# luotuoqingshan/SDPLRPlus.jl

Hardware: AMD Instinct MI355X
Metric: augmented-Lagrangian iters/sec + HBM GB/s, MaxCut n=1e5 r=32 (higher is better)
Workload: dtype f64

## Files before the change

sdplrplus.jl_amd/cabi.py:

```python
from __future__ import annotations

import ctypes as C
import os
from typing import Optional, Tuple

import numpy as np

OK = 0
ERR_INVALID_ARG = -1
ERR_HIP = -2
ERR_NOT_DESCENT = -3
ERR_STATE = -4
ERR_NO_DEVICE = -5
ERR_ALLOC = -6
ERR_UNSERVED = -7
MAJOR_RESUME = 2

F_RT, F_GT, F_DIRT, F_LBFGS_S, F_LBFGS_Y, F_SCRATCH = 0, 1, 2, 100, 200, 300
(V_LAMBDA, V_LAMBDA_UB, V_B, V_Y, V_PV_RAW, V_PV_LB, V_PV, V_A_RD, V_A_DD, V_LBFGS_RHO, V_LBFGS_A,
 V_UVT, V_TRIU_S_NZVAL, V_S_NZVAL, V_SCRATCH) = range(15)
STAT_NAMES = ("graph_captures", "graph_capture_failures", "graph_capture_skipped", "graph_batches",
              "eager_batches", "lanczos_graph_replays", "lanczos_eager_rounds", "inner_iterations",
              "resident_loops", "resident_lanczos", "resident_fg", "resident_shared_launches", "p_less_loops",
              "group_launch_loops", "ring_history_loops", "ring_materializations")
S_SIGMA, S_OBJ, S_LBFGS_LATEST = 0, 1, 2

_i32, _i64, _f64, _vp = C.c_int32, C.c_int64, C.c_double, C.c_void_p
_pi32, _pi64, _pf64 = C.POINTER(C.c_int32), C.POINTER(C.c_int64), C.POINTER(C.c_double)



class FgItem(C.Structure):
    _fields_ = [("s", _vp), ("normC", _f64), ("normb", _f64), ("gtol_relative", _i32), ("ptol_relative", _i32),
                ("lagrangian", _f64), ("grad_norm", _f64), ("primal_vio_norm", _f64), ("obj", _f64), ("status", _i32)]


class MajorItem(C.Structure):
    _fields_ = [("s", _vp), ("normC", _f64), ("normb", _f64), ("gtol_relative", _i32), ("ptol_relative", _i32),
                ("use_armijo", _i32), ("update_lambda", _i32), ("sigma", _f64), ("cur_gtol", _f64), ("fprec_eps", _f64),
                ("max_local_iters", _i64), ("time_budget_s", _f64), ("lagrangian", _f64), ("grad_norm", _f64),
                ("primal_vio_norm", _f64), ("last_alpha", _f64), ("obj", _f64), ("iters_done", _i64),
                ("exit_reason", _i32), ("status", _i32)]


class DualItem(C.Structure):
    _fields_ = [("s", _vp), ("trace_bound", _f64), ("iter", _i64), ("v0", _pf64), ("y_out", _pf64),
                ("dual_value", _f64), ("mineig", _f64), ("status", _i32)]


SIGNATURES = {
    "device_count": [_pi32],
    "set_device": [_i32],
    "last_error": [_vp],
    "version": [],
    "device_synchronize": [],
    "warmup": [_i32],
    "trim_pools": [],
    "create": [_i64, _i64, _i64, _i64, C.POINTER(_vp)],
    "set_sparse": [_vp, _i64, _i64, _pi64, _pi64, _pf64, _pf64, _pi64, _i64, _pi64, _pi64, _i64,
                   _pi64, _pi64, _pi64],
    "set_sparse_coo": [_vp, _i64, _i64, _pi64, _pi64, _pi64, _pf64, _pi64],
    "get_layout": [_vp, _i32, _pi64, _pf64, _i64, _pi64],
    "add_symlowrank": [_vp, _i64, _i64, _i64, _pf64, _pf64],
    "finalize": [_vp],
    "destroy": [_vp],
    "reset_rank": [_vp, _i64],
    "set_factor": [_vp, _i32, _pf64],
    "get_factor": [_vp, _i32, _pf64],
    "set_vec": [_vp, _i32, _pf64, _i64],
    "get_vec": [_vp, _i32, _pf64, _i64],
    "set_scalar": [_vp, _i32, _f64],
    "get_scalar": [_vp, _i32, _pf64],
    "get_dims": [_vp, _pi64, _pi64, _pi64, _pi64, _pi64, _pi64, _pi64],
    "A": [_vp, _i32, _i32, _i32],
    "At_preprocess": [_vp],
    "At_left": [_vp, _i32, _i32],
    "At_right": [_vp, _pf64, _pf64, _i64],
    "At_right_device": [_vp, _vp, _vp, _i64],
    "get_stats": [_vp, _pi64, _i32, _pi32],
    "S_eigval": [_vp, _i64, _i32, _i64, _f64, _i64, _pf64, _pf64, _pi64, _pi64],
    "factor_dot": [_vp, _i32, _i32, _pf64],
    "f": [_vp, _pf64],
    "g": [_vp],
    "fg": [_vp, _f64, _f64, _i32, _i32, _pf64, _pf64, _pf64],
    "lbfgs_clear": [_vp],
    "lbfgs_dir": [_vp, _i32, _pf64],
    "descent_fallback": [_vp],
    "lbfgs_update": [_vp, _f64],
    "linesearch": [_vp, _f64, _pf64, _pf64],
    "linesearch_armijo": [_vp, _f64, _pf64, _pf64],
    "axpy_R": [_vp, _f64],
    "norms": [_vp, _f64, _f64, _i32, _i32, _pf64, _pf64],
    "update_lambda": [_vp],
    "inner_loop": [_vp, _f64, _f64, _i32, _i32, _i32, _f64, _f64, _i64, _f64, _pf64, _pf64, _pf64,
                   _pf64, _pi64, _pi32],
    "major_iteration": [_vp, _f64, _f64, _i32, _i32, _i32, _i32, _f64, _f64, _f64, _i64, _f64, _pf64, _pf64, _pf64,
                        _pf64, _pi64, _pi32],
    "batch_fg": [_i32, C.POINTER(FgItem)],
    "batch_major_iteration": [_i32, C.POINTER(MajorItem)],
    "batch_dual_obj": [_i32, C.POINTER(DualItem)],
    "lanczos": [_vp, _i64, _pf64, _pf64, _pf64, _pi64],
    "tridiag_mineig": [_pf64, _pf64, _i64, _pf64],
    "approx_mineigval_lanczos": [_vp, _i64, _pf64, _pf64],
    "dual_obj": [_vp, _f64, _i64, _pf64, _pf64, _pf64],
    "profile_enable": [_vp, _i32],
    "profile_filter": [_vp, C.c_char_p],
    "profile_count": [_vp, _pi32],
# ... 420 lines not shown
```

sdplrplus.jl_amd/csrc/k_dense.h:

```cpp
#pragma once
#include "common.h"

struct FactorArena {
  double* base;
  long long stride;
  int h;
};
#define AS_R 0
#define AS_G 1
#define AS_D 2
#define AS_S0 3

#ifdef SDPLR_NO_NT
__device__ __forceinline__ double2 ldnt2(const double* p, long long i) { return reinterpret_cast<const double2*>(p)[i]; }
__device__ __forceinline__ void stnt2(double* p, long long i, double2 v) { reinterpret_cast<double2*>(p)[i] = v; }
#else
typedef double sdplr_d2 __attribute__((ext_vector_type(2)));
__device__ __forceinline__ double2 ldnt2(const double* p, long long i) {
  const sdplr_d2 t = __builtin_nontemporal_load(reinterpret_cast<const sdplr_d2*>(p) + i);
  double2 o;
  o.x = t.x;
  o.y = t.y;
  return o;
}
// ... 181 lines not shown
      return;
    }
    c.iters = iters + 1;
    c.lastval = Lcur;
  }
  int ord[H];
  {
    int j = latest - 1;
#pragma unroll
    for (int i = 0; i < H; i++) {
      ord[i] = j;
      j = (j <= 0) ? H - 1 : j - 1;
    }
  }
  double Sg_s[H], Yg_s[H];
#pragma unroll
  for (int l = 0; l < H; l++) {
    Sg_s[l] = c.Sg[l];
    Yg_s[l] = c.Yg[l];
  }
  double al_s[H], ga_s[H];
#pragma unroll
  for (int l = 0; l < H; l++) {
    al_s[l] = c.c_alpha[l];
    ga_s[l] = c.c_gamma[l];
  }
  if (do_coeff) {
    double SYp[H][H], YYp[H][H], Sgp[H], Ygp[H], rhop[H];
#pragma unroll
    for (int a = 0; a < H; a++) {
      Sgp[a] = c.Sg[ord[a]];
      Ygp[a] = c.Yg[ord[a]];
      rhop[a] = c.rho[ord[a]];
#pragma unroll
      for (int b = 0; b < H; b++) {
        SYp[a][b] = c.SY[ord[a] * SDPLR_HMAX + ord[b]];
        YYp[a][b] = c.YY[ord[a] * SDPLR_HMAX + ord[b]];
      }
    }
    double al[H], ga[H];
#pragma unroll
    for (int i = 0; i < H; i++) {
      double sq = Sgp[i];
#pragma unroll
      for (int k = 0; k < i; k++) sq -= al[k] * SYp[i][k];
      al[i] = rhop[i] * sq;
    }
#pragma unroll
    for (int i = H - 1; i >= 0; i--) {
      double yr = Ygp[i];
#pragma unroll
      for (int k = 0; k < H; k++) yr -= al[k] * YYp[i][k];
#pragma unroll
      for (int k = H - 1; k > i; k--) yr += ga[k] * SYp[k][i];
      const double beta = rhop[i] * yr;
      ga[i] = al[i] - beta;
    }
#pragma unroll
    for (int i = 0; i < H; i++) {
      c.a[ord[i]] = al[i];
      c.c_alpha[ord[i]] = al[i];
      c.c_gamma[ord[i]] = ga[i];
#pragma unroll
      for (int l = 0; l < H; l++)
        if (ord[i] == l) {
          al_s[l] = al[i];
          ga_s[l] = ga[i];
        }
    }
  }
  if (desc_mode) {
    const double g = grel ? gnorm * normC : gnorm;
    double d = norms ? nrm0 : g * g;
#pragma unroll
    for (int l = 0; l < H; l++) d -= al_s[l] * Yg_s[l];
#pragma unroll
    for (int l = 0; l < H; l++) d += ga_s[l] * Sg_s[l];
    if (desc_mode == 1) d = -d;
    c.descent = d;
    c.fallback = (isnan(d) || d >= 0.0) ? 1 : 0;
  }
}

__device__ __forceinline__ void lbfgs_boundary_body(DevCtrl* __restrict__ c, int h, int jfixed, int fin_mode, int do_loop, int do_coeff, int nb_partials, const double* __restrict__ partials, int desc_mode, double* __restrict__ pv_raw, int m) {
  __shared__ SeamLds gd;
  const int tid = threadIdx.x, wave = tid >> 6, lane = tid & 63;
#ifdef SDPLR_STAMPS
  const unsigned long long st0 = __builtin_amdgcn_s_memtime();
#endif
  const int gp = c->gram_pending, np = c->norms_pending;
  const int op = c->obj_pending;
  static_assert(sizeof(DevCtrl) / 8 <= 1024, "one word of the control block per thread");
  const unsigned long long cw = reinterpret_cast<const unsigned long long*>(c)[min(tid, (int)(sizeof(DevCtrl) / 8) - 1)];
  if (wave >= 14) {
    const int nbp = (wave == 14) ? c->nb_gnorm : c->nb_pvnorm;
    const double* p = slot_partials(partials, wave == 14 ? SLOT_GNORM2 : SLOT_PVNORM2);
    const double2* p2 = reinterpret_cast<const double2*>(p);
    double2 v[8];
#pragma unroll
    for (int u = 0; u < 8; u++) v[u] = p2[lane + 64 * u];
    double t = 0.0;
#pragma unroll
    for (int u = 0; u < 8; u++) {
      const int i = 2 * (lane + 64 * u);
      t += (i < nbp) ? v[u].x : 0.0;
      t += (i + 1 < nbp) ? v[u].y : 0.0;
    }
    for (int i = lane + 1024; i < nbp; i += 64) t += p[i];
    t = wave_sum(t);
    if (lane == 0) gd.nrm[wave - 14] = t;
  } else if (fin_mode != 0) {
    const int np2 = (nb_partials + 1) >> 1;
    for (int s0 = wave; s0 < 5 * h; s0 += 28) {
      const int s1 = s0 + 14;
      const bool two = s1 < 5 * h;
      const double2* pa = reinterpret_cast<const double2*>(slot_partials(partials, SLOT_GRAM + (s0 / h) * SDPLR_HMAX + s0 % h));
      const double2* pb = two ? reinterpret_cast<const double2*>(slot_partials(partials, SLOT_GRAM + (s1 / h) * SDPLR_HMAX + s1 % h)) : pa;
      double ta = 0.0, tb = 0.0;
#pragma unroll 4
      for (int i = lane; i < np2; i += 64) {
        const double2 a = pa[i], b = pb[i];
        const bool hi = 2 * i + 1 < nb_partials;
        ta += a.x;
        ta += hi ? a.y : 0.0;
        tb += b.x;
        tb += hi ? b.y : 0.0;
      }
      ta = wave_sum(ta);
      tb = wave_sum(tb);
      if (lane == 0) {
        gd.red[(s0 / h) * SDPLR_HMAX + s0 % h] = ta;
        if (two) gd.red[(s1 / h) * SDPLR_HMAX + s1 % h] = tb;
      }
    }
  }
  if (tid < (int)(sizeof(DevCtrl) / 8)) reinterpret_cast<unsigned long long*>(&gd.c)[tid] = cw;
  const bool fin = (fin_mode == 2) || (fin_mode == 1 && gp);
  const bool norms = np != 0;
  if (!fin && !do_coeff && !do_loop && !norms && !op) return;
  __syncthreads();
  if (tid == 0 && op) {
    gd.c.obj = gd.c.obj_next;
    gd.c.obj_pending = 0;
    if (pv_raw != nullptr) pv_raw[m] = gd.c.obj_next;
  }
  if (tid == 0 && fin_mode == 1 && gd.c.ring_on) {
    if (gp) {
      gd.c.ring_alpha[gd.c.latest % h] = gd.c.alpha;
      gd.c.ring_k = (gd.c.ring_k + 1) % (h + 1);
      gd.c.ring_n = min(gd.c.ring_n + 1, h);
    } else if (gd.c.reldelta_exit) {
      gd.c.ring_unc = 1;
    }
  }
#ifdef SDPLR_STAMPS
  const unsigned long long st1 = __builtin_amdgcn_s_memtime();
#endif
  if (tid == 0) {
    switch (h) {
      case 1: seam_serial_small<1>(gd, jfixed, fin_mode, do_loop, do_coeff, fin, norms, desc_mode); break;
      case 2: seam_serial_small<2>(gd, jfixed, fin_mode, do_loop, do_coeff, fin, norms, desc_mode); break;
      case 3: seam_serial_small<3>(gd, jfixed, fin_mode, do_loop, do_coeff, fin, norms, desc_mode); break;
      case 4: seam_serial_small<4>(gd, jfixed, fin_mode, do_loop, do_coeff, fin, norms, desc_mode); break;
      default: seam_serial(gd, h, jfixed, fin_mode, do_loop, do_coeff, fin, norms, desc_mode);
    }
  }
  __syncthreads();
#ifdef SDPLR_STAMPS
  const unsigned long long st2 = __builtin_amdgcn_s_memtime();
#endif
  {
    const unsigned long long* src = reinterpret_cast<const unsigned long long*>(&gd.c);
    unsigned long long* dst = reinterpret_cast<unsigned long long*>(c);
    for (int t = tid; t < (int)(sizeof(DevCtrl) / 8); t += 1024) dst[t] = src[t];
  }
#ifdef SDPLR_STAMPS
  asm volatile("s_waitcnt vmcnt(0)" ::: "memory");
  const unsigned long long st3 = __builtin_amdgcn_s_memtime();
  if (tid == 0 && do_loop && (gd.c.iters % 64) == 33) {
    printf("[seam] loads+sums %llu  serial %llu  store %llu (s_memtime ticks)\n", st1 - st0, st2 - st1, st3 - st2);
  }
#endif
}
__global__ void __launch_bounds__(1024)
k_lbfgs_boundary(DevCtrl* __restrict__ c, int h, int jfixed, int fin_mode, int do_loop, int do_coeff,
                 int nb_partials, const double* __restrict__ partials, int desc_mode, double* __restrict__ pv_raw = nullptr,
                 int m = 0) {
  lbfgs_boundary_body(c, h, jfixed, fin_mode, do_loop, do_coeff, nb_partials, partials, desc_mode, pv_raw, m);
}

template <int HM, bool NTH>
__device__ __forceinline__ void lbfgs_dir_body(const DevCtrl* __restrict__ c, FactorArena A, long long N, int h, int negate, int check_done, double* __restrict__ partials, int inline_fallback) {
  __shared__ double sh[8];
  const int dn = check_done ? c->done : 0;
  double* G = aslot(A, AS_G);
  double* dir = aslot(A, AS_D);
  const int latest = c->latest;
  const int fb = inline_fallback ? c->fallback : 0;
  int order[HM];
  double ca[HM], cg[HM];
  {
    int j = latest - 1;
#pragma unroll
    for (int i = 0; i < HM; i++) {
      order[i] = j;
      if (i < h) {
        ca[i] = c->c_alpha[j];
        cg[i] = c->c_gamma[j];
      } else {
        ca[i] = 0.0;
        cg[i] = 0.0;
      }
      j = (j <= 0) ? h - 1 : j - 1;
    }
  }
  double* ynext = (h > 0 && inline_fallback != 2) ? aslot(A, as_y0(A) + (latest % h)) : nullptr;
  const double sgn = negate ? -1.0 : 1.0;
  if (dn) return;
  double desc = 0.0;
  const long long N2 = N >> 1;
  const long long stride = (long long)gridDim.x * SDPLR_NT;
  const double* yp[HM];
  const double* sp_[HM];
#pragma unroll
  for (int k = 0; k < HM; k++) {
    const int slot = (k < h) ? order[k] : 0;
    yp[k] = (h > 0) ? aslot(A, as_y0(A) + slot) : G;
    sp_[k] = (h > 0) ? aslot(A, AS_S0 + slot) : G;
  }
  for (long long i = (long long)blockIdx.x * SDPLR_NT + threadIdx.x; i < N2; i += stride) {
    const double2 g = ldnt2(G, i);
    double2 yv[HM], sv[HM];
#pragma unroll
    for (int k = 0; k < HM; k++) {
      if constexpr (NTH) {
        yv[k] = ldnt2(yp[k], i);
        sv[k] = ldnt2(sp_[k], i);
      } else {
        yv[k] = reinterpret_cast<const double2*>(yp[k])[i];
        sv[k] = reinterpret_cast<const double2*>(sp_[k])[i];
      }
    }
    double2 r = g;
#pragma unroll
    for (int k = 0; k < HM; k++) {
      r.x -= ca[k] * yv[k].x;
      r.y -= ca[k] * yv[k].y;
    }
#pragma unroll
    for (int k = HM - 1; k >= 0; k--) {
      r.x += cg[k] * sv[k].x;
      r.y += cg[k] * sv[k].y;
    }
    double2 d;
    d.x = sgn * r.x;
    d.y = sgn * r.y;
    if (fb) {
      d.x = -g.x;
      d.y = -g.y;
      reinterpret_cast<double2*>(G)[i] = d;
    }
    reinterpret_cast<double2*>(dir)[i] = d;
    if (ynext) {
      double2 ng;
      ng.x = -g.x;
      ng.y = -g.y;
      stnt2(ynext, i, ng);
    }
    desc += d.x * g.x + d.y * g.y;
  }
  if ((N & 1) && blockIdx.x == 0 && threadIdx.x == 0) {
// ... 434 lines not shown
```

sdplrplus.jl_amd/csrc/k_group.h:

```cpp
#pragma once
#include "k_dense.h"
#include "k_scalar.h"
#include "k_sparse.h"

struct GrpSeamArgs {
  DevCtrl* c;
  int h, jfixed, fin_mode, do_loop, do_coeff, nb_partials;
  const double* partials;
  int desc_mode, m;
  double* pv_raw;
};
struct GrpDirArgs {
  const DevCtrl* c;
  FactorArena A;
  long long N;
  int h, negate, check_done, inline_fallback;
  double* partials;
};
struct GrpSddmmArgs {
  DevSparse sp;
  DevLowRank lr;
  int m, r;
  const double *U, *V;
  double *A_RD, *A_DD, *lr_part, *partials;
  const DevCtrl* c;
};
struct GrpSumsArgs {
  int nout, nb, nb_c, m, n_extra;
  const double* lr_part;
  double *W, *red2;
  const int* extra;
  const double *lam, *pv_raw, *A_RD, *A_DD;
  double* partials;
  const DevCtrl* c;
};
struct GrpLsArgs {
  DevCtrl* c;
  int m, gid_g, n_extra, nb, lr_ST, r, check_done, lr_tail, lr_n;
  const int* extra;
  double *A_RD, *A_DD;
  const double *lam, *lam_ub;
  double* pv_raw;
  const double* lb;
  double *pv, *y;
  const int* lr_col_gid;
  const double* lr_D;
  double *lrW, *lrWS;
  const double* partials;
  const int *lr_mat_ptr, *lr_mat_gid;
  const double* red2;
  ExtraHead eh;
};
struct GrpStepArgs {
  DevSparse sp;
  DevCtrl* c;
  double* R;
  const double* D;
  long long N;
  int nb_ax, nb_c, m, n_extra, nb_gnorm;
  const int* extra;
  double* pv_raw;
  const double *A_RD, *A_DD, *lb;
  double *pv, *y;
  const double *lam, *lam_ub;
  double* partials;
};
struct GrpSpmmArgs {
  DevSparse sp;
  DevLowRank lr;
  FactorArena A;
  const double* X;
  double* Y;
  int r, slot, nb_long, h;
  double scale;
  const double* WS;
  double* partials;
  DevCtrl* c;
  const double* D;
};

__global__ void __launch_bounds__(1024) k_grp_boundary(const GrpSeamArgs* __restrict__ tab) {
  const GrpSeamArgs a = tab[blockIdx.y];
  lbfgs_boundary_body(a.c, a.h, a.jfixed, a.fin_mode, a.do_loop, a.do_coeff, a.nb_partials, a.partials, a.desc_mode, a.pv_raw, a.m);
}
template <int HM>
__global__ void __launch_bounds__(SDPLR_NT) k_grp_dir(const GrpDirArgs* __restrict__ tab) {
  const GrpDirArgs a = tab[blockIdx.y];
  lbfgs_dir_body<HM, false>(a.c, a.A, a.N, a.h, a.negate, a.check_done, a.partials, a.inline_fallback);
}
template <int LPR, int VEC, int LRN>
__global__ void __launch_bounds__(SDPLR_NT) k_grp_sddmm_edge(const GrpSddmmArgs* __restrict__ tab) {
  const GrpSddmmArgs a = tab[blockIdx.y];
  sddmm_edge_body<LPR, VEC, LRN>(a.sp, a.m, a.U, a.V, a.r, a.A_RD, a.A_DD, a.lr, a.lr_part, a.partials, a.c);
}
__global__ void __launch_bounds__(SDPLR_NT) k_grp_edge_sums(const GrpSumsArgs* __restrict__ tab) {
  const GrpSumsArgs a = tab[blockIdx.y];
  edge_sums_body(a.nout, a.nb, a.lr_part, a.W, a.red2, a.nb_c, a.m, a.n_extra, a.extra, a.lam, a.pv_raw, a.A_RD, a.A_DD, a.partials, a.c);
}
__global__ void __launch_bounds__(SDPLR_LSF_NT) k_grp_ls_solve_fast(const GrpLsArgs* __restrict__ tab) {
  const GrpLsArgs a = tab[blockIdx.y];
  ls_solve_fast_body(a.c, a.m, a.gid_g, a.n_extra, a.extra, a.nb, a.A_RD, a.A_DD, a.lam, a.lam_ub, a.pv_raw, a.lb, a.pv, a.y, a.lr_ST, a.r,
                     a.lr_col_gid, a.lr_D, a.lrW, a.lrWS, a.partials, a.check_done, a.lr_tail, a.lr_n, a.lr_mat_ptr, a.lr_mat_gid, a.red2,
                     a.eh);
}
__global__ void __launch_bounds__(SDPLR_NT) k_grp_edge_step(const GrpStepArgs* __restrict__ tab) {
  const GrpStepArgs a = tab[blockIdx.y];
  edge_step_body(a.sp, a.c, a.R, a.D, a.N, a.nb_ax, a.nb_c, a.m, a.n_extra, a.extra, a.pv_raw, a.A_RD, a.A_DD, a.lb, a.pv, a.y, a.lam,
                 a.lam_ub, a.partials, a.nb_gnorm);
}
template <int LPR, int VEC>
__global__ void __launch_bounds__(SDPLR_NT) k_grp_spmm_both_upd(const GrpSpmmArgs* __restrict__ tab) {
  const GrpSpmmArgs a = tab[blockIdx.y];
  spmm_both_upd_body<LPR, VEC, 4, false>(a.sp, a.X, a.Y, a.r, a.scale, a.lr, a.WS, a.slot, a.partials, a.c, a.nb_long, a.A, a.h, a.D, nullptr);
}
__global__ void __launch_bounds__(64) k_grp_poll(const DevCtrl* const* __restrict__ ctrls, int count, int* __restrict__ out) {
  for (int b = threadIdx.x; b < count; b += 64) out[b] = ctrls[b]->done;
}
```

sdplrplus.jl_amd/csrc/k_sparse.h:

```cpp
#pragma once
#include "common.h"
#include "k_dense.h"
#include "k_scalar.h"

struct DevSparse {
  int n, nnzT, nnzS, nnzAgg, n_sparse;
  const int *triu_colptr, *triu_rowval, *triu_colidx;
  const int *colptr, *rowval, *mapped;
  double *nzval, *triu_nzval;
  const int *matptr, *nzind, *gids;
  const double *nzval_one, *nzval_two;
  const int *tptr, *tmat;
  const double* tval;
  int n_short, n_chunks, n_long, n_short_blocks;
  const int *short_ids, *chunk_beg, *chunk_end, *long_ids, *long_chunk_ptr;
  double *chunk_partial0, *chunk_partial1;
  double *UVt0, *UVt1;
  int n_long_rows, long_thresh;
  const int* long_rows;
  const int* q_gid;
  const double* q_two;
  const double* q_rec;
  const int* s_gid;
  const double* s_one;
  int big_gid;
  const int* own_pos;
  const double* own_one;
  int n_big_pos;
  const int* big_pos;
  const double* big_one;
};

struct DevLowRank {
  int n_lr, ST;
  const double* Bcat;
  const double* Dcat;
  const int* col_gid;
  const int* mat_ptr;
  const int* mat_gid;
};

template <int VEC> struct vecd;
template <> struct vecd<1> { double v[1]; };
template <> struct vecd<2> { double v[2]; };

template <int VEC>
__device__ __forceinline__ vecd<VEC> ldrow(const double* __restrict__ p) {
  vecd<VEC> o;
  if constexpr (VEC == 2) {
    const double2 t = *reinterpret_cast<const double2*>(p);
    o.v[0] = t.x;
    o.v[VEC - 1] = t.y;
  } else {
    o.v[0] = *p;
  }
  return o;
}
template <int VEC>
__device__ __forceinline__ void strow(double* __restrict__ p, const vecd<VEC>& o) {
  if constexpr (VEC == 2) {
    double2 t;
    t.x = o.v[0];
    t.y = o.v[VEC - 1];
    *reinterpret_cast<double2*>(p) = t;
  } else {
    *p = o.v[0];
  }
}

template <int VEC>
__device__ __forceinline__ void strow_nt(double* __restrict__ p, const vecd<VEC>& o) {
  if constexpr (VEC == 2) {
    typedef double d2 __attribute__((ext_vector_type(2)));
    d2 t;
    t.x = o.v[0];
    t.y = o.v[VEC - 1];
    __builtin_nontemporal_store(t, reinterpret_cast<d2*>(p));
  } else {
    __builtin_nontemporal_store(o.v[0], p);
  }
}

#ifndef SDPLR_STEP_TR
// ... 867 lines not shown
          }
          if (HMU > 0 && !upd) {
            vecd<VEC> go;
#pragma unroll
            for (int q = 0; q < VEC; q++) go.v[q] = 0.0;
#pragma unroll
            for (int l = 0; l < HMU; l++)
              if (l == jslot) go = yv[u][l];
#pragma unroll
            for (int q = 0; q < VEC; q++) go.v[q] = gs * go.v[q];
            if (gold_in_G) strow<VEC>(rowat(Yj, offc), go);
          }
          if (HMU > 0 && upd) {
            vecd<VEC> sn, yn;
#pragma unroll
            for (int q = 0; q < VEC; q++) yn.v[q] = 0.0;
#pragma unroll
            for (int l = 0; l < HMU; l++)
              if (l == jslot) yn = yv[u][l];
#pragma unroll
            for (int q = 0; q < VEC; q++) {
              sn.v[q] = a * d.v[q];
              yn.v[q] = gs * yn.v[q] + g.v[q];
            }
            strow<VEC>(rowat(Sj, offc), sn);
            strow<VEC>(rowat(Yj, offc), yn);
#pragma unroll
            for (int l = 0; l < HMU; l++)
              if (l < h) {
                const vecd<VEC> sl = (l == jslot) ? sn : sv[u][l];
                const vecd<VEC> yl = (l == jslot) ? yn : yv[u][l];
                double q0 = 0.0, q1 = 0.0, q2 = 0.0, q3 = 0.0, q4 = 0.0;
#pragma unroll
                for (int q = 0; q < VEC; q++) {
                  q0 += sn.v[q] * yl.v[q];
                  q1 += sl.v[q] * yn.v[q];
                  q2 += yn.v[q] * yl.v[q];
                  q3 += sl.v[q] * g.v[q];
                  q4 += yl.v[q] * g.v[q];
                }
                double* ac = accl + threadIdx.x;
                (void)__hip_atomic_fetch_add(ac + (0 * HMU + l) * SDPLR_NT, q0, __ATOMIC_RELAXED, __HIP_MEMORY_SCOPE_WORKGROUP);
                (void)__hip_atomic_fetch_add(ac + (1 * HMU + l) * SDPLR_NT, q1, __ATOMIC_RELAXED, __HIP_MEMORY_SCOPE_WORKGROUP);
                (void)__hip_atomic_fetch_add(ac + (2 * HMU + l) * SDPLR_NT, q2, __ATOMIC_RELAXED, __HIP_MEMORY_SCOPE_WORKGROUP);
                (void)__hip_atomic_fetch_add(ac + (3 * HMU + l) * SDPLR_NT, q3, __ATOMIC_RELAXED, __HIP_MEMORY_SCOPE_WORKGROUP);
                (void)__hip_atomic_fetch_add(ac + (4 * HMU + l) * SDPLR_NT, q4, __ATOMIC_RELAXED, __HIP_MEMORY_SCOPE_WORKGROUP);
              }
          }
          if (HMU > 0 && LPR < 64) break;
        }
      }
    }
  }
  if (dn) return;
  if constexpr (HMU > 0) {
    __syncthreads();
    if (upd) {
      const int wave = threadIdx.x >> 6, wl = threadIdx.x & 63;
      for (int k = wave; k < 5 * HMU; k += SDPLR_NT / 64) {
        double t = 0.0;
#pragma unroll
        for (int i = 0; i < SDPLR_NT / 64; i++) t += accl[k * SDPLR_NT + wl + 64 * i];
        t = wave_sum(t);
        const int q = k / HMU, l = k % HMU;
        if (wl == 0 && l < h) slot_partials(partials, SLOT_GRAM + q * SDPLR_HMAX + l)[blockIdx.x] = t;
      }
      if (blockIdx.x == 0 && threadIdx.x == 0) c->gram_pending = 1;
    }
  }
  block_sum<2>(red, sh);
  if (threadIdx.x == 0) {
    slot_partials(partials, SLOT_GNORM2)[blockIdx.x] = red[0];
    if (COMMIT) {
      slot_partials(partials, SLOT_PVNORM2)[blockIdx.x] = red[1];
      if (blockIdx.x == 0) {
        c->norms_pending = 1;
        c->nb_gnorm = gridDim.x;
        c->nb_pvnorm = gridDim.x;
      }
    }
  }
}

template <int LPR, int VEC, int HMU, bool PB = false>
__global__ void __launch_bounds__(SDPLR_NT)
k_fast_step_ring(int n, int m, DevFast ff, double* __restrict__ R, const double* __restrict__ W, int r,
                 double* __restrict__ yvec, const double* __restrict__ lam, const double* __restrict__ lam_ub,
                 double* __restrict__ pv_raw, const double* __restrict__ lb, double* __restrict__ pv,
                 const double* __restrict__ A_RD, const double* __restrict__ A_DD, double* __restrict__ partials,
                 DevCtrl* __restrict__ c, int check_done, FactorArena A, int h, int nb_ls,
                 double* __restrict__ P = nullptr, DevLowRank lr = DevLowRank{}, const double* __restrict__ WS = nullptr) {
  static_assert(HMU >= 1, "the ring form rides the fused update");
  __shared__ double sh[2 * (SDPLR_NT / 64)];
  __shared__ double shl[10 * (SDPLR_NT / 64)];
  extern __shared__ double accl[];
  const int dn = check_done ? c->done : 0;
  constexpr int G = SDPLR_NT / LPR;
  const int lane = threadIdx.x % LPR;
  const long long total = (long long)gridDim.x * G;
  const double sigma = c->sigma;
  const int latest = c->latest, rk = c->ring_k, rn = c->ring_n, rj0 = c->ring_j0;
  double a, yg = 1.0;
  bool upd;
  if constexpr (PB) {
    a = c->alpha;
    yg = yvec[ff.gid_g];
    upd = c->reldelta_exit == 0;
  } else {
    const double obj0 = c->obj, amax = c->alpha_max, last = c->lastval, feps = c->fprec_eps;
    double s10[10];
    {
      constexpr int PT = 2;
      double2 v[10][PT];
      const int ncols = (nb_ls + 2 * SDPLR_NT - 1) / (2 * SDPLR_NT);
#pragma unroll
      for (int q = 0; q < PT; q++) {
        const int i = (int)threadIdx.x + SDPLR_NT * q;
        if (q < ncols) {
#pragma unroll
          for (int k = 0; k < 8; k++) v[k][q] = reinterpret_cast<const double2*>(slot_partials(partials, SLOT_LS + k))[i];
          v[8][q] = reinterpret_cast<const double2*>(slot_partials(partials, SLOT_PD))[i];
          v[9][q] = reinterpret_cast<const double2*>(slot_partials(partials, SLOT_DW))[i];
        } else {
#pragma unroll
          for (int k = 0; k < 10; k++) v[k][q].x = v[k][q].y = 0.0;
        }
      }
#pragma unroll
      for (int k = 0; k < 10; k++) {
        s10[k] = 0.0;
#pragma unroll
        for (int q = 0; q < PT; q++) {
          const int i = 2 * ((int)threadIdx.x + SDPLR_NT * q);
          s10[k] += (i < nb_ls) ? v[k][q].x : 0.0;
          s10[k] += (i + 1 < nb_ls) ? v[k][q].y : 0.0;
        }
      }
    }
    block_sum<10>(s10, shl);
    const double g_rd = s10[8] + s10[8], g_dd = s10[9];
    double bq[5];
    bq[0] = obj0 - s10[0] + sigma * s10[1] / 2;
    bq[1] = g_rd - s10[2] + sigma * s10[3];
    bq[2] = g_dd - s10[4] + sigma * s10[5] / 2;
    bq[3] = sigma * s10[6];
    bq[4] = sigma * s10[7] / 2;
    double al = 0.0, f = bq[0];
    const int rc = quartic_argmin(bq, amax, &al, &f);
    if (rc != 0) {
      if (blockIdx.x == 0 && threadIdx.x == 0 && !dn) {
        c->err = rc;
        c->done = 1;
      }
      return;
    }
    const double rel_delta = (last - f) / fmax(1.0, fmax(fabs(f), fabs(last)));
    upd = !(rel_delta < feps);
    a = al;
    if (blockIdx.x == 0 && threadIdx.x == 0 && !dn) {
      for (int k = 0; k < 5; k++) c->biquad[k] = bq[k];
      c->alpha = al;
      c->L = f;
      c->reldelta_exit = upd ? 0 : 1;
      const_cast<double*>(A_RD)[m] = g_rd;
      const_cast<double*>(A_DD)[m] = g_dd;
      c->obj_next = obj0 + al * (al * g_dd + g_rd);
      c->obj_pending = 1;
      c->pv2_extra = 0.0;
    }
  }
  const int jslot = latest % h;
  const int nv = h - 1;
  constexpr int HO = HMU > 1 ? HMU - 1 : 1;
  const double* gp[HMU];
  const double* dp[HO];
  double ra[HO];
  int lsl[HO];
  gp[0] = ring_G(A, rk, rj0);
#pragma unroll
  for (int i = 0; i < HO; i++) {
    int l = (latest - 1 - i) % h;
    if (l < 0) l += h;
    lsl[i] = l;
    const double r0 = c->ring_alpha[l];
    ra[i] = (i < rn) ? r0 : 1.0;
    if (i >= nv) {
      dp[i] = gp[0];
      if (i + 1 < HMU) gp[i + 1] = gp[0];
    } else if (i < rn) {
      dp[i] = ring_D(A, ring_back(rk, 1 + i, h), rj0);
      if (i + 1 < HMU) gp[i + 1] = ring_G(A, ring_back(rk, 1 + i, h), rj0);
    } else {
      dp[i] = aslot(A, AS_S0 + l);
      if (i + 1 < HMU) gp[i + 1] = aslot(A, as_y0(A) + l);
    }
  }
  double* const D = ring_D(A, rk, rj0);
  double* const Gnew = ring_G(A, ring_back(rk, -1, h), rj0);
  double red[2] = {0.0, 0.0};
  const int ch0 = lane * VEC;
#pragma unroll
  for (int k = 0; k < 5 * HMU; k++) accl[k * SDPLR_NT + threadIdx.x] = 0.0;
  constexpr int TR = LPR < SDPLR_STEP_TR ? LPR : SDPLR_STEP_TR;
  const long long ntiles = ((long long)n + TR - 1) / TR;
  for (long long tile = (long long)blockIdx.x * G + threadIdx.x / LPR; tile < ntiles; tile += total) {
    const long long j0 = tile * TR;
    const int nrows = (int)min((long long)TR, (long long)n - j0);
    if (dn) return;
    double djl = 0.0, djo = 0.0;
    if (lane < nrows) {
      const long long j = j0 + lane;
      const int e0 = ff.drow_ptr[j], e1 = ff.drow_ptr[j + 1];
      for (int e = e0; e < e1; e++) {
        const int k = ff.drow_gid[e];
        if (!PB) djo += ff.drow_val[e] * yvec[k];
        const double v = pv_raw[k] + a * (a * A_DD[k] + A_RD[k]);
        double yk;
        if (k < m) {
          yk = -fmin(lam_ub[k], lam[k] - sigma * v);
          const double pc = fmax(v, lb[k]);
          pv[k] = pc;
          red[1] += pc * pc;
        } else {
          yk = 1.0;
          c->obj = v;
        }
        djl += ff.drow_val[e] * yk;
        yvec[k] = yk;
        pv_raw[k] = v;
      }
    }
    for (int i0 = 0; i0 < nrows; i0 += 2) {
      vecd<VEC> xx[2], pq[2], dd[2], ww[2], gv[2][HMU], dv[2][HO];
      double dj[2], dq[2];
      unsigned off[2];
#pragma unroll
      for (int u = 0; u < 2; u++) {
        const int i = min(i0 + u, nrows - 1);
        const long long j = j0 + i;
        dj[u] = __shfl(djl, i, LPR);
        dq[u] = __shfl(djo, i, LPR);
        off[u] = (unsigned)(((unsigned long long)j * (unsigned)r + (unsigned)ch0) * 8ull);
#pragma unroll
        for (int q = 0; q < VEC; q++) xx[u].v[q] = pq[u].v[q] = dd[u].v[q] = ww[u].v[q] = 0.0;
#pragma unroll
        for (int l = 0; l < HMU; l++)
#pragma unroll
          for (int q = 0; q < VEC; q++) gv[u][l].v[q] = 0.0;
#pragma unroll
        for (int l = 0; l < HO; l++)
#pragma unroll
          for (int q = 0; q < VEC; q++) dv[u][l].v[q] = 0.0;
        if (ch0 < r) {
          xx[u] = ldrow<VEC>(rowat(R, off[u]));
          if (PB) pq[u] = ldrow<VEC>(rowat(P, off[u]));
          dd[u] = ldrow<VEC>(rowat(D, off[u]));
          ww[u] = ldrow<VEC>(rowat(W, off[u]));
#pragma unroll
          for (int l = 0; l < HMU; l++) gv[u][l] = ldrow_nt<VEC>(rowat(gp[l], off[u]));
#pragma unroll
          for (int l = 0; l < HO; l++) dv[u][l] = ldrow_nt<VEC>(rowat(dp[l], off[u]));
        }
      }
#pragma unroll
      for (int u = 0; u < 2; u++) {
        if (i0 + u >= nrows) break;
        if (ch0 >= r) continue;
        vecd<VEC> x = xx[u];
        const vecd<VEC> d = dd[u], w = ww[u], go = gv[u][0];
        vecd<VEC> g;
        if constexpr (PB) {
          vecd<VEC> pp = pq[u];
#pragma unroll
          for (int q = 0; q < VEC; q++) {
            x.v[q] += a * d.v[q];
            pp.v[q] += a * w.v[q];
            g.v[q] = pp.v[q] * yg + x.v[q] * dj[u];
          }
          const long long jrow = j0 + i0 + u;
          for (int cc = 0; cc < lr.ST; cc++) {
            const double bb = lr.Bcat[(long long)cc * n + jrow];
            const vecd<VEC> ws = ldrow<VEC>(WS + (long long)cc * r + ch0);
#pragma unroll
            for (int q = 0; q < VEC; q++) g.v[q] += ws.v[q] * bb;
          }
#pragma unroll
          for (int q = 0; q < VEC; q++) {
            g.v[q] *= 2.0;
            red[0] += g.v[q] * g.v[q];
          }
          strow<VEC>(rowat(P, off[u]), pp);
        } else {
#pragma unroll
          for (int q = 0; q < VEC; q++) {
            const double xo = x.v[q];
            x.v[q] += a * d.v[q];
            const double t = a * w.v[q] + (x.v[q] * dj[u] - xo * dq[u]);
            g.v[q] = go.v[q] + 2.0 * t;
            red[0] += g.v[q] * g.v[q];
          }
        }
#ifdef SDPLR_RING_NT_R
        strow_nt<VEC>(rowat(R, off[u]), x);
#else
        strow<VEC>(rowat(R, off[u]), x);
#endif
#ifdef SDPLR_RING_NT_G
        strow_nt<VEC>(rowat(Gnew, off[u]), g);
#else
        strow<VEC>(rowat(Gnew, off[u]), g);
#endif
        if (upd) {
          vecd<VEC> sn, yn;
#pragma unroll
          for (int q = 0; q < VEC; q++) {
            sn.v[q] = a * d.v[q];
            yn.v[q] = g.v[q] - go.v[q];
          }
          double* ac = accl + threadIdx.x;
#pragma unroll
          for (int i = 0; i < HO; i++)
            if (i < nv) {
              double q0 = 0.0, q1 = 0.0, q2 = 0.0, q3 = 0.0, q4 = 0.0;
#pragma unroll
              for (int q = 0; q < VEC; q++) {
                const double sl = ra[i] * dv[u][i].v[q];
                const double yn1 = gv[u][i + 1 < HMU ? i + 1 : i].v[q];
                const double yl = (i < rn) ? gv[u][i].v[q] - yn1 : yn1;
                q0 += sn.v[q] * yl;
                q1 += sl * yn.v[q];
                q2 += yn.v[q] * yl;
                q3 += sl * g.v[q];
                q4 += yl * g.v[q];
              }
              const int l = lsl[i];
              (void)__hip_atomic_fetch_add(ac + (0 * HMU + l) * SDPLR_NT, q0, __ATOMIC_RELAXED, __HIP_MEMORY_SCOPE_WORKGROUP);
              (void)__hip_atomic_fetch_add(ac + (1 * HMU + l) * SDPLR_NT, q1, __ATOMIC_RELAXED, __HIP_MEMORY_SCOPE_WORKGROUP);
              (void)__hip_atomic_fetch_add(ac + (2 * HMU + l) * SDPLR_NT, q2, __ATOMIC_RELAXED, __HIP_MEMORY_SCOPE_WORKGROUP);
              (void)__hip_atomic_fetch_add(ac + (3 * HMU + l) * SDPLR_NT, q3, __ATOMIC_RELAXED, __HIP_MEMORY_SCOPE_WORKGROUP);
              (void)__hip_atomic_fetch_add(ac + (4 * HMU + l) * SDPLR_NT, q4, __ATOMIC_RELAXED, __HIP_MEMORY_SCOPE_WORKGROUP);
            }
          {
            double q0 = 0.0, q2 = 0.0, q3 = 0.0, q4 = 0.0;
#pragma unroll
            for (int q = 0; q < VEC; q++) {
              q0 += sn.v[q] * yn.v[q];
              q2 += yn.v[q] * yn.v[q];
              q3 += sn.v[q] * g.v[q];
              q4 += yn.v[q] * g.v[q];
            }
            (void)__hip_atomic_fetch_add(ac + (0 * HMU + jslot) * SDPLR_NT, q0, __ATOMIC_RELAXED, __HIP_MEMORY_SCOPE_WORKGROUP);
            (void)__hip_atomic_fetch_add(ac + (1 * HMU + jslot) * SDPLR_NT, q0, __ATOMIC_RELAXED, __HIP_MEMORY_SCOPE_WORKGROUP);
            (void)__hip_atomic_fetch_add(ac + (2 * HMU + jslot) * SDPLR_NT, q2, __ATOMIC_RELAXED, __HIP_MEMORY_SCOPE_WORKGROUP);
            (void)__hip_atomic_fetch_add(ac + (3 * HMU + jslot) * SDPLR_NT, q3, __ATOMIC_RELAXED, __HIP_MEMORY_SCOPE_WORKGROUP);
            (void)__hip_atomic_fetch_add(ac + (4 * HMU + jslot) * SDPLR_NT, q4, __ATOMIC_RELAXED, __HIP_MEMORY_SCOPE_WORKGROUP);
          }
        }
      }
    }
  }
  if (dn) return;
  __syncthreads();
  if (upd) {
    const int wave = threadIdx.x >> 6, wl = threadIdx.x & 63;
    for (int k = wave; k < 5 * HMU; k += SDPLR_NT / 64) {
      double t = 0.0;
#pragma unroll
      for (int i = 0; i < SDPLR_NT / 64; i++) t += accl[k * SDPLR_NT + wl + 64 * i];
      t = wave_sum(t);
      const int q = k / HMU, l = k % HMU;
      if (wl == 0 && l < h) slot_partials(partials, SLOT_GRAM + q * SDPLR_HMAX + l)[blockIdx.x] = t;
    }
    if (blockIdx.x == 0 && threadIdx.x == 0) c->gram_pending = 1;
  }
  block_sum<2>(red, sh);
  if (threadIdx.x == 0) {
    slot_partials(partials, SLOT_GNORM2)[blockIdx.x] = red[0];
    slot_partials(partials, SLOT_PVNORM2)[blockIdx.x] = red[1];
    if (blockIdx.x == 0) {
      c->norms_pending = 1;
      c->nb_gnorm = gridDim.x;
      c->nb_pvnorm = gridDim.x;
    }
  }
}

template <int LPR, int VEC>
__global__ void __launch_bounds__(SDPLR_NT)
k_spmm_fast(DevSparse sg, int m, DevFast ff, const double* __restrict__ R, const double* __restrict__ D,
            const double* __restrict__ P, double* __restrict__ W, int r, const double* __restrict__ lam,
            const double* __restrict__ pv_raw, double* __restrict__ A_RD, double* __restrict__ A_DD,
            double* __restrict__ partials, const DevCtrl* __restrict__ c, int check_done) {
  __shared__ double sh[10 * (SDPLR_NT / 64)];
  if (check_done && c->done) return;
  constexpr int G = SDPLR_NT / LPR;
  const int lane = threadIdx.x % LPR;
  const long long total = (long long)gridDim.x * G;
  const double sigma = c->sigma;
  double acc[10];
#pragma unroll
  for (int k = 0; k < 10; k++) acc[k] = 0.0;
  for (long long j = (long long)blockIdx.x * G + threadIdx.x / LPR; j < sg.n; j += total) {
    const int beg = sg.colptr[j], end = sg.colptr[j + 1];
    double rd = 0.0, dd = 0.0;
    for (int chb = 0; chb < r; chb += LPR * VEC) {
      const int ch = chb + lane * VEC;
      const bool act = ch < r;
      vecd<VEC> xr, xd, w;
#pragma unroll
      for (int k = 0; k < VEC; k++) xr.v[k] = xd.v[k] = w.v[k] = 0.0;
      if (act) {
        xr = ldrow<VEC>(R + j * r + ch);
        xd = ldrow<VEC>(D + j * r + ch);
      }
      for (int base = beg; base < end; base += LPR) {
        const int cnt = min(LPR, end - base);
        const int my_i = (lane < cnt) ? sg.rowval[base + lane] : 0;
        const double my_v = (lane < cnt) ? sg.nzval[base + lane] : 0.0;
        for (int k0 = 0; k0 < cnt; k0 += 8) {
          vecd<VEC> x[8];
          double v[8];
#pragma unroll
          for (int q = 0; q < 8; q++) {
            const int src = min(k0 + q, LPR - 1);
            const long long i = __shfl(my_i, src, LPR);
            v[q] = __shfl(my_v, src, LPR);
            if (act && k0 + q < cnt) {
              x[q] = ldrow<VEC>(D + i * r + ch);
            } else {
#pragma unroll
              for (int k = 0; k < VEC; k++) x[q].v[k] = 0.0;
              v[q] = 0.0;
            }
          }
#pragma unroll
          for (int q = 0; q < 8; q++)
#pragma unroll
            for (int k = 0; k < VEC; k++) w.v[k] += x[q].v[k] * v[q];
        }
      }
#pragma unroll
      for (int k = 0; k < VEC; k++) {
        rd += xr.v[k] * xd.v[k];
        dd += xd.v[k] * xd.v[k];
        acc[8] += xr.v[k] * w.v[k];
        acc[9] += xd.v[k] * w.v[k];
      }
      if (act) strow<VEC>(W + j * r + ch, w);
    }
    rd = group_sum<LPR>(rd);
    dd = group_sum<LPR>(dd);
    if (lane == 0)
      for (int e = ff.drow_ptr[j]; e < ff.drow_ptr[j + 1]; e++) {
        const int k = ff.drow_gid[e];
        const double v = ff.drow_val[e];
        const double q1 = v * (rd + rd), q2 = v * dd;
        A_RD[k] = q1;
        A_DD[k] = q2;
        if (k < m) {
          const double l = lam[k], nq0 = pv_raw[k];
          acc[0] += l * nq0;
          acc[1] += nq0 * nq0;
          acc[2] += l * q1;
          acc[3] += nq0 * q1;
          acc[4] += (l - sigma * nq0) * q2;
          acc[5] += q1 * q1;
          acc[6] += q1 * q2;
// ... 1279 lines not shown
```

sdplrplus.jl_amd/csrc/sdplr_hip.hip:

```cpp
#include "../../include/sdplr_hip.h"

#include <hip/hip_runtime.h>

#include <algorithm>
#include <atomic>
#include <chrono>
#include <cmath>
#include <cstddef>
#include <cstdio>
#include <cstdlib>
#include <cstring>
#include <limits>
#include <map>
#include <memory>
#include <mutex>
#include <shared_mutex>
#include <string>
#include <thread>
#include <unordered_map>
#include <utility>
#include <vector>

#include "common.h"
#include "k_dense.h"
// ... 25 lines not shown
  return ms;
}

struct LowRankHost {
  int64_t gid, s;
  std::vector<double> B, D;
};

struct ProfEntry {
  int64_t launches = 0;
  double ms = 0.0;
};

}

struct BandHost {
  bool ok = false, pal = false;
  int NB = 0, NC = 0, BW = 0, CH = 0;
  size_t n_groups = 0;
  std::vector<int> fcp, frv;
  std::vector<int> blk_slot, slot_g, diagpos;
  std::vector<uint4> cw;
  std::vector<int4> pos;
  std::vector<double> palv;
  int env_min_n = 0, env_bw = 0, env_ch = 0, env_nc = 0;
  bool env_no_band = false, env_no_pal = false;
};

struct sdplr_hip_solver {
  int64_t n = 0, m = 0, r = 0, h = 0;
  bool finalized = false;
  hipStream_t stream = nullptr;
  std::string err;

  bool have_sparse = false;
  int64_t n_sparse = 0, nnzT = 0, nnzS = 0, nnzAgg = 0;
  std::vector<int> h_matptr, h_nzind, h_gids, h_tcp, h_trv, h_fcp, h_frv, h_mapped;
  std::vector<double> h_one, h_two;
  std::vector<LowRankHost> h_lr;

  struct UploadArena {
    bool on = false;
    char* dev = nullptr;
    char* host = nullptr;
    size_t cap = 0, used = 0;
    char* zdev = nullptr;
    size_t zcap = 0, zused = 0;
  } up;
  int device = -1;
  std::vector<void*> allocs;
  DevSparse sp{};
  DevLowRank lr{};
  bool all_covered = false;
  bool fast = false;
  DevFast ff{};
  DevSparse sp_fast{};
  DevSparse spg{};
  DevTile tile{};
  bool edge = false;
  const int* edge_extra = nullptr;
  ExtraHead edge_extra_head{}, extra_head{};
  int n_edge_extra = 0, nb_edge = 1;
  bool edge_lr_fused = false;
  DevBand band{};
  bool use_band = false;
  std::unique_ptr<BandHost> band_host;
  std::thread band_thread;
  int nb_tile = 0, nb_step = 1, tile_blocks = 512;
  bool use_tile = false;
  bool tiles_deferred = false;
  bool tile_attr_done = false;
  bool tile_panels = false;
  bool lit = false;
  double *lit_rho = nullptr, *lit_a = nullptr;
  bool no_lshead = false;
  bool no_team = false;
  double* rs_xch = nullptr;
  int rs_ell_parts = 1;
  int rs_ell_part_sl[SDPLR_RS_TEAM_MAX + 1] = {0, 0, 0, 0, 0};
  bool no_pdrop = false;
  bool pdrop_now = false;
  bool no_ring = false;
  bool ring_on = false, ring_now = false;
  int ring_k = 0, ring_n = 0, ring_unc = 0, ring_latest = 0, ring_j0 = 0;
  double ring_alpha[SDPLR_HMAX] = {};
  bool G_consistent = false;
  int64_t G_age = 0;
  int dirt_from = -1;
  bool no_updfuse = false;
  int gram_nb = 1;
  bool force_graph = false;
  bool no_lrfuse = false;
  bool dot_descent = false;
  int tile_lpr = 0;
  std::vector<int> h_gptr, h_gcol;
  std::vector<double> h_gval;
  std::vector<void*> tile_allocs;
  bool fast_singleton = false;
  bool rs_ok = false;
  double* rs_rowvec = nullptr;
  const int* rs_row_k = nullptr;
  const double* rs_row_v = nullptr;
  RsEll rs_ell{};
  size_t rs_ell_pair_lines = 0;
  const int* extra_slots = nullptr;
  int n_extra = 0;
  FactorArena arena{};
  long long N = 0;
  double *lambda = nullptr, *lambda_ub = nullptr, *b = nullptr, *y = nullptr, *pv_raw = nullptr,
         *pv_lb = nullptr, *pv = nullptr, *A_RD = nullptr, *A_DD = nullptr;
  DevCtrl* ctrl = nullptr;
  DevCtrl* hc = nullptr;
  bool hc_valid = false;
  DevCtrl* snap[2] = {nullptr, nullptr};
  hipEvent_t snap_ev[2] = {nullptr, nullptr};
  double* partials = nullptr;
  double *lz_buf[3] = {nullptr, nullptr, nullptr}, *lz_v0 = nullptr, *lz_alpha = nullptr, *lz_beta = nullptr;
  int64_t lz_cap = 0;
  double *lr_part = nullptr, *lr_W = nullptr, *lr_WS = nullptr, *lr_coef = nullptr, *lr_btx_part = nullptr;
  double* red10 = nullptr;
  int nb_lr = 1;

  int LPR = 1, VEC = 1, HM = 4;
  int nb_lzv = 1;
  int lz_graph_reps = 0;
  int nb_upd = 1;
  int nb_dense = 1, nb_m = 1, nb_sddmm = 1, nb_spmm = 1, nb_spmv = 1, nb_nnzT = 1, nb_nnzS = 1, nb_n = 1;

  hipGraphExec_t graph_exec[5] = {nullptr, nullptr, nullptr, nullptr, nullptr};
  int graph_iters = 8;
  bool graph_disabled = false;
  hipGraphExec_t lz_graph = nullptr;

  bool gram_dirty = false, sg_stale = false, ynext_pending = false;
  bool P_valid = false, S_stale = false;
  bool S_from_y = true;
  bool lz_band_now = false;
  int64_t P_age = 0;

  double* scratchF[2] = {nullptr, nullptr};
  double* scratchV = nullptr;
  int64_t st_captures = 0, st_capture_failed = 0, st_capture_skipped = 0, st_graph_batches = 0,
          st_eager_batches = 0, st_lz_graph = 0, st_lz_eager = 0, st_iters = 0, st_rs_loops = 0, st_rs_lz = 0, st_rs_fg = 0, st_rs_shared = 0, st_pdrop = 0, st_grp_loops = 0, st_ring_loops = 0, st_ring_materialized = 0;

  bool prof_on = false;
  std::string prof_filter;
  std::vector<std::string> prof_names;
  std::map<std::string, int> prof_index;
  std::vector<ProfEntry> prof;
  struct Pending { int id; hipEvent_t a, b; };
  std::vector<Pending> prof_pending;
  std::vector<hipEvent_t> ev_pool;
};

namespace {
using S = sdplr_hip_solver;
inline int dev_of(const S* s) { return s ? s->device : -1; }
void ensure_S(S* s);

int fail(S* s, int code, const std::string& msg) {
  if (s) s->err = msg; else g_err = msg;
  return code;
}
#define HIPCK(s, call)                                                                      \
  do {                                                                                      \
    hipError_t e__ = (call);                                                                \
    if (e__ != hipSuccess)                                                                  \
      return fail((s), SDPLR_ERR_HIP, std::string(#call) + ": " + hipGetErrorString(e__));  \
  } while (0)
#define NEED_FINAL(s)                                                            \
  do {                                                                           \
    if (!(s)) return fail(nullptr, SDPLR_ERR_INVALID_ARG, "null handle");        \
    if (!(s)->finalized) return fail((s), SDPLR_ERR_STATE, "not finalized");     \
  } while (0)
int ensure_dirt(S* s);
int ensure_canonical(S* s);
int blocks_for(long long work, int per_block, int cap);
#define NEED_FINAL_RW(s)                                   \
  do {                                                     \
    NEED_FINAL(s);                                         \
    (s)->hc_valid = false;                                 \
    (s)->G_consistent = false;                             \
    if ((s)->ring_on) {                                    \
      const int rc_r__ = ensure_canonical(s);              \
      if (rc_r__) return rc_r__;                           \
    }                                                      \
    if ((s)->dirt_from >= 0) {                             \
      const int rc_d__ = ensure_dirt(s);                   \
      if (rc_d__) return rc_d__;                           \
    }                                                      \
  } while (0)

#define NEED_FINAL_RW_KEEP_HISTORY(s)                      \
  do {                                                     \
    NEED_FINAL(s);                                         \
    (s)->hc_valid = false;                                 \
    (s)->G_consistent = false;                             \
  } while (0)

int have_device() {
  int c = 0;
  if (hipGetDeviceCount(&c) != hipSuccess) return 0;
  return c;
}

int host_threads() {
  static const int n = [] {
    int k = (int)std::thread::hardware_concurrency();
    if (const char* e = getenv("SDPLR_HIP_HOST_THREADS")) k = atoi(e);
    return std::max(1, std::min(k, 8));
  }();
  return n;
}
template <typename F>
void parallel_for(int64_t n_items, int64_t min_per_thread, F&& body) {
  const int64_t nt = std::max<int64_t>(1, std::min<int64_t>(host_threads(), n_items / std::max<int64_t>(min_per_thread, 1)));
  if (nt <= 1) { body((int64_t)0, n_items); return; }
  std::vector<std::thread> th;
  for (int64_t t = 0; t < nt; t++) {
    const int64_t b = n_items * t / nt, e = n_items * (t + 1) / nt;
    th.emplace_back([&body, b, e] { body(b, e); });
  }
  for (auto& x : th) x.join();
}

struct DevPool {
  std::mutex mu;
  std::map<std::pair<int, size_t>, std::vector<void*>> free_blocks;
  std::unordered_map<void*, std::pair<int, size_t>> live;
  std::vector<void*> pinned_free;
  std::vector<void*> pinned_chunks_free;
  std::map<int, std::vector<hipStream_t>> streams_free;
  std::map<int, std::vector<hipEvent_t>> events_free;
  size_t cached = 0;
  struct Slab {
    int dev;
    char* base;
    size_t size, used, n_carved, n_cached;
  };
  std::vector<Slab> slabs;
// ... 1355 lines not shown
    const int len = s->h_matptr[k + 1] - s->h_matptr[k];
    if (len <= SHORT_MAX) { short_ids.push_back((int)k); continue; }
    long_ids.push_back((int)k);
    for (int bgn = s->h_matptr[k]; bgn < s->h_matptr[k + 1]; bgn += CHUNK) {
      chunk_beg.push_back(bgn);
      chunk_end.push_back(std::min(bgn + CHUNK, s->h_matptr[k + 1]));
    }
    long_chunk_ptr.push_back((int)chunk_beg.size());
  }
  sp.n_short = (int)short_ids.size(); sp.n_chunks = (int)chunk_beg.size(); sp.n_long = (int)long_ids.size();
  sp.n_short_blocks = (sp.n_short + SDPLR_NT - 1) / SDPLR_NT;
  {
    std::vector<char> cov(m + 1, 0);
    for (int g : s->h_gids) cov[g] = 1;
    for (auto& L : s->h_lr) cov[L.gid] = 1;
    s->all_covered = std::all_of(cov.begin(), cov.end(), [](char c) { return c != 0; });
  }
  lap("transpose + reduction plan");
#define UP(field, vec) if ((rc = upload(s, &sp.field, vec))) return rc
  UP(triu_colptr, s->h_tcp); UP(triu_rowval, s->h_trv); UP(triu_colidx, colidx);
  UP(colptr, s->h_fcp); UP(rowval, s->h_frv); UP(mapped, s->h_mapped);
  UP(matptr, s->h_matptr); UP(nzind, s->h_nzind); UP(gids, s->h_gids);
  UP(nzval_one, s->h_one); UP(nzval_two, s->h_two);
  UP(tptr, tptr); UP(tmat, tmat); UP(tval, tval);
  UP(short_ids, short_ids); UP(chunk_beg, chunk_beg); UP(chunk_end, chunk_end);
  UP(long_ids, long_ids); UP(long_chunk_ptr, long_chunk_ptr);
#undef UP
  auto plan_long = [&](const std::vector<int>& ptr, DevSparse& dst) -> int {
    std::vector<int> deg(n);
    for (int64_t j = 0; j < n; j++) deg[j] = ptr[j + 1] - ptr[j];
    const long long mean3 = n > 0 ? 3LL * ptr[n] / n : 0;
    int thresh = (int)std::min<long long>(std::max<long long>(64, mean3), 1 << 30);
    if (const char* e = getenv("SDPLR_HIP_HUB_THRESH")) thresh = std::max(8, atoi(e));
    std::vector<int> rows;
    for (int64_t j = 0; j < n; j++)
      if (deg[j] > thresh) rows.push_back((int)j);
    dst.n_long_rows = (int)rows.size();
    dst.long_thresh = thresh;
    return upload(s, &dst.long_rows, rows);
  };
  lap("uploads (layout)");
  if ((rc = plan_long(s->h_fcp, sp))) return rc;
  if ((rc = dzero(s, &sp.nzval, s->nnzS))) return rc;
  if ((rc = dzero(s, &sp.triu_nzval, s->nnzT))) return rc;
  if ((rc = dzero(s, &sp.UVt0, s->nnzT))) return rc;
  if ((rc = dzero(s, &sp.UVt1, s->nnzT))) return rc;
  if ((rc = dzero(s, &sp.chunk_partial0, sp.n_chunks))) return rc;
  if ((rc = dzero(s, &sp.chunk_partial1, sp.n_chunks))) return rc;
  DevLowRank& lr = s->lr;
  lr.n_lr = (int)s->h_lr.size();
  {
    std::vector<double> Bcat, Dcat;
    std::vector<int> col_gid, mat_ptr(1, 0), mat_gid;
    for (auto& L : s->h_lr) {
      Bcat.insert(Bcat.end(), L.B.begin(), L.B.end());
      Dcat.insert(Dcat.end(), L.D.begin(), L.D.end());
      for (int64_t t = 0; t < L.s; t++) col_gid.push_back((int)L.gid);
      mat_ptr.push_back((int)col_gid.size());
      mat_gid.push_back((int)L.gid);
    }
    lr.ST = (int)col_gid.size();
    if ((rc = upload(s, &lr.Bcat, Bcat))) return rc;
    if ((rc = upload(s, &lr.Dcat, Dcat))) return rc;
    if ((rc = upload(s, &lr.col_gid, col_gid))) return rc;
    if ((rc = upload(s, &lr.mat_ptr, mat_ptr))) return rc;
    if ((rc = upload(s, &lr.mat_gid, mat_gid))) return rc;
  }
  if ((rc = dzero(s, &s->lambda, m))) return rc;
  if ((rc = dzero(s, &s->b, m))) return rc;
  if ((rc = dzero(s, &s->pv, m))) return rc;
  if ((rc = dzero(s, &s->y, m + 1))) return rc;
  if ((rc = dzero(s, &s->pv_raw, m + 1))) return rc;
  if ((rc = dzero(s, &s->A_RD, m + 1))) return rc;
  if ((rc = dzero(s, &s->A_DD, m + 1))) return rc;
  {
    std::vector<double> inf(m, std::numeric_limits<double>::infinity()), ninf(m, -std::numeric_limits<double>::infinity());
    const double *ub = nullptr, *lb = nullptr;
    if ((rc = upload(s, &ub, inf))) return rc;
    if ((rc = upload(s, &lb, ninf))) return rc;
    s->lambda_ub = const_cast<double*>(ub);
    s->pv_lb = const_cast<double*>(lb);
  }
  if ((rc = dzero(s, &s->partials, (size_t)SDPLR_NSLOT * SDPLR_MAXNB))) return rc;
  for (int k = 0; k < 3; k++)
    if ((rc = dzero(s, &s->lz_buf[k], n + 64))) return rc;
  if ((rc = dzero(s, &s->lz_v0, n))) return rc;
  s->nb_lr = 256;
  if ((rc = dzero(s, &s->lr_btx_part, (size_t)std::max(lr.ST, 1) * SDPLR_MAXNB))) return rc;
  if ((rc = dzero(s, &s->lr_coef, 2 * (size_t)std::max(lr.ST, 1)))) return rc;
  if ((rc = dzero(s, &s->red10, 16))) return rc;
  {
    DevCtrl* d = nullptr;
    if ((rc = dalloc(s, &d, 1))) return rc;
    s->ctrl = d;
    HIPCK(s, pool_host_ctrl((void**)&s->hc));
    memset(s->hc, 0, sizeof(DevCtrl));
    s->hc->sigma = 2.0;
    s->hc->alpha_max = 1.0;
    s->hc->latest = (int)s->h;
    HIPCK(s, hipMemcpyAsync(s->ctrl, s->hc, sizeof(DevCtrl), hipMemcpyHostToDevice, s->stream));
    HIPCK(s, hipStreamSynchronize(s->stream));
    for (int k = 0; k < 2; k++) {
      HIPCK(s, pool_host_ctrl((void**)&s->snap[k]));
      HIPCK(s, pool_event(&s->snap_ev[k]));
    }
  }
  lap("vectors + control block");
  s->dot_descent = getenv("SDPLR_HIP_DOT_DESCENT") != nullptr;
  s->lit = s->h > SDPLR_HMAX;
  if (s->lit) {
    s->dot_descent = true;
    if ((rc = dzero(s, &s->lit_rho, (size_t)s->h))) return rc;
    if ((rc = dzero(s, &s->lit_a, (size_t)s->h))) return rc;
  }
  if (const char* e = getenv("SDPLR_HIP_GRAPH_ITERS")) s->graph_iters = std::max(1, std::min(atoi(e), 64));
  s->no_lrfuse = getenv("SDPLR_HIP_NO_LRFUSE") != nullptr;
  s->force_graph = getenv("SDPLR_HIP_FORCE_GRAPH") != nullptr;
  s->no_updfuse = getenv("SDPLR_HIP_NO_UPDFUSE") != nullptr;
  s->no_pdrop = getenv("SDPLR_HIP_NO_PDROP") != nullptr;
  s->no_lshead = getenv("SDPLR_HIP_NO_LSHEAD") != nullptr;
  s->no_ring = getenv("SDPLR_HIP_NO_RING") != nullptr;
  s->tile_panels = getenv("SDPLR_HIP_TILE_PANELS") != nullptr;
  if (s->have_sparse && getenv("SDPLR_HIP_NO_FAST") == nullptr) {
    std::vector<int> general;
    for (int64_t k = 0; k < s->n_sparse; k++) {
      bool diag_only = true;
      for (int e = s->h_matptr[k]; e < s->h_matptr[k + 1] && diag_only; e++)
        diag_only = (s->h_trv[s->h_nzind[e]] == colidx[s->h_nzind[e]]);
      if (!diag_only) general.push_back((int)k);
    }
    if (general.size() == 1) {
      const int kg = general[0];
      std::vector<int> g_ptr(n + 1, 0), g_col;
      std::vector<double> g_val;
      const int eb = s->h_matptr[kg], ee = s->h_matptr[kg + 1];
      bool ascending = true;
      for (int e = eb + 1; e < ee && ascending; e++) ascending = s->h_nzind[e] > s->h_nzind[e - 1];
      if (ascending) {
        for (int e = eb; e < ee; e++) {
          const int q = s->h_nzind[e], i = s->h_trv[q], j = colidx[q];
          g_ptr[i + 1]++;
          if (i != j) g_ptr[j + 1]++;
        }
        for (int64_t i = 0; i < n; i++) g_ptr[i + 1] += g_ptr[i];
        g_col.resize(g_ptr[n]);
        g_val.resize(g_ptr[n]);
        std::vector<int> fillg(g_ptr.begin(), g_ptr.end() - 1);
        for (int e = eb; e < ee; e++) {
          const int q = s->h_nzind[e], i = s->h_trv[q], j = colidx[q];
          if (i != j) { const int pos = fillg[j]++; g_col[pos] = i; g_val[pos] = s->h_one[e]; }
        }
        for (int e = eb; e < ee; e++) {
          const int q = s->h_nzind[e], i = s->h_trv[q], j = colidx[q];
          const int pos = fillg[i]++; g_col[pos] = j; g_val[pos] = s->h_one[e];
        }
      } else {
        struct Ent { int i, j; double v; };
        std::vector<Ent> ents;
        for (int e = eb; e < ee; e++) {
          const int q = s->h_nzind[e], i = s->h_trv[q], j = colidx[q];
          ents.push_back({i, j, s->h_one[e]});
          if (i != j) ents.push_back({j, i, s->h_one[e]});
        }
        std::stable_sort(ents.begin(), ents.end(), [](const Ent& a, const Ent& b) { return a.i != b.i ? a.i < b.i : a.j < b.j; });
        for (size_t t = 0; t < ents.size(); t++) {
          if (t > 0 && ents[t].i == ents[t - 1].i && ents[t].j == ents[t - 1].j) { g_val.back() += ents[t].v; continue; }
          g_col.push_back(ents[t].j);
          g_val.push_back(ents[t].v);
          g_ptr[ents[t].i + 1]++;
        }
        for (int64_t i = 0; i < n; i++) g_ptr[i + 1] += g_ptr[i];
      }
      lap("A_g CSR");
      std::vector<int> d_ptr(n + 1, 0);
      for (int64_t k = 0; k < s->n_sparse; k++)
        if ((int)k != kg)
          for (int e = s->h_matptr[k]; e < s->h_matptr[k + 1]; e++) d_ptr[s->h_trv[s->h_nzind[e]] + 1]++;
      for (int64_t i = 0; i < n; i++) d_ptr[i + 1] += d_ptr[i];
      std::vector<int> d_gid(d_ptr[n]), fillp(d_ptr.begin(), d_ptr.end() - 1);
      std::vector<double> d_val(d_ptr[n]);
      for (int64_t k = 0; k < s->n_sparse; k++)
        if ((int)k != kg)
          for (int e = s->h_matptr[k]; e < s->h_matptr[k + 1]; e++) {
            const int pos = fillp[s->h_trv[s->h_nzind[e]]]++;
            d_gid[pos] = s->h_gids[k];
            d_val[pos] = s->h_one[e];
          }
      std::vector<int> diagpos(n, -1);
      for (int64_t j = 0; j < n; j++)
        for (int q = s->h_tcp[j]; q < s->h_tcp[j + 1]; q++)
          if (s->h_trv[q] == (int)j) diagpos[j] = q;
      std::vector<int> f_short, f_cb, f_ce, f_long, f_lcp(1, 0);
      for (int64_t k = 0; k < s->n_sparse; k++) {
        if ((int)k == kg) continue;
        const int len = s->h_matptr[k + 1] - s->h_matptr[k];
        if (len <= SHORT_MAX) { f_short.push_back((int)k); continue; }
        f_long.push_back((int)k);
        for (int bgn = s->h_matptr[k]; bgn < s->h_matptr[k + 1]; bgn += CHUNK) {
          f_cb.push_back(bgn);
          f_ce.push_back(std::min(bgn + CHUNK, s->h_matptr[k + 1]));
        }
        f_lcp.push_back((int)f_cb.size());
      }
      s->sp_fast = sp;
// ... 106 lines not shown
      for (size_t t = 0; t < 4; t++) s->edge_extra_head.k[t] = t < extra.size() ? extra[t] : 0;
      s->n_edge_extra = (int)extra.size();
      bool all_diag = true;
      {
        std::vector<char> has(n, 0);
        for (int64_t j = 0; j < n; j++)
          for (int q = s->h_tcp[j]; q < s->h_tcp[j + 1]; q++)
            if (s->h_trv[q] == (int)j) has[j] = 1;
        all_diag = std::all_of(has.begin(), has.end(), [](char c) { return c != 0; });
      }
      s->edge_lr_fused = lr.ST == 1 && all_diag && !s->no_lrfuse;
      s->edge = true;
    }
  }
  lap("classification / edge plan");
  s->use_band = false;
  s->band_host.reset(new BandHost());
  s->band_host->fcp = s->h_fcp;
  s->band_host->frv = std::move(s->h_frv);
  {
    BandHost& H = *s->band_host;
    auto envi = [](const char* k) { const char* e = getenv(k); return e ? std::max(1, atoi(e)) : 0; };
    H.env_min_n = envi("SDPLR_HIP_LZBAND_MIN_N"); H.env_bw = envi("SDPLR_HIP_LZBAND_BW");
    H.env_ch = envi("SDPLR_HIP_LZBAND_CH"); H.env_nc = envi("SDPLR_HIP_LZBAND_NC");
    H.env_no_band = getenv("SDPLR_HIP_NO_LZBAND") != nullptr; H.env_no_pal = getenv("SDPLR_HIP_NO_LZPAL") != nullptr;
  }
  const bool band_possible = s->have_sparse && s->nnzS > 0 && !s->band_host->env_no_band &&
                             n >= (s->band_host->env_min_n > 0 ? s->band_host->env_min_n : (1 << 14));
  if (getenv("SDPLR_HIP_BAND_SYNC") != nullptr || !band_possible) {
    band_host(s, *s->band_host);
  } else {
    S* sp_ = s;
    BandHost* hp_ = s->band_host.get();
    s->band_thread = std::thread([sp_, hp_] { band_host(sp_, *hp_); });
  }
  lap("band plan (started)");
  if ((rc = alloc_factors(s))) return rc;
  lap("factors");
  s->nb_m = blocks_for(m + 1, SDPLR_NT, 256);
  s->nb_spmv = blocks_for(n, SDPLR_NT / 8, 768);
  s->nb_nnzT = blocks_for(s->nnzT, SDPLR_NT, 4096);
  s->nb_nnzS = blocks_for(s->nnzS, SDPLR_NT, 4096);
  s->nb_n = blocks_for(n, SDPLR_NT, 1024);
  lap("before commit");
  if ((rc = arena_commit(s))) return rc;
  s->up.on = false;
  lap("arena commit");
  if ((rc = dzero(s, &s->lr_part, (size_t)std::max(s->nb_lr, SDPLR_MAXNB) * 2 * std::max(lr.ST, 1) * s->r))) return rc;
  if ((rc = dzero(s, &s->lr_W, (size_t)2 * std::max(lr.ST, 1) * s->r))) return rc;
  if ((rc = dzero(s, &s->lr_WS, (size_t)std::max(lr.ST, 1) * s->r))) return rc;
  if (s->tiles_deferred && !s->rs_ok) {
    s->tiles_deferred = false;
    if ((rc = build_tiles(s))) return rc;
  }
  std::vector<int>().swap(s->h_nzind); std::vector<int>().swap(s->h_trv); std::vector<int>().swap(s->h_frv);
  std::vector<int>().swap(s->h_mapped); std::vector<double>().swap(s->h_one); std::vector<double>().swap(s->h_two);
  for (auto& L : s->h_lr) { std::vector<double>().swap(L.B); }
  lap("rank-sized scratch");
  HIPCK(s, hipStreamSynchronize(s->stream));
  lap("final sync");
  s->finalized = true;
  return SDPLR_OK;
}

int32_t sdplr_hip_destroy(S* s) {
  ApiShared api_guard(dev_of(s));
  if (!s) return SDPLR_OK;
  if (s->band_thread.joinable()) s->band_thread.join();
  if (s->stream) (void)hipStreamSynchronize(s->stream);
  for (auto& p : s->prof_pending) { (void)hipEventDestroy(p.a); (void)hipEventDestroy(p.b); }
  for (auto e : s->ev_pool) (void)hipEventDestroy(e);
  for (void* p : s->allocs) pool_free(p);
  if (s->arena.base) pool_free(s->arena.base);
  if (s->lz_alpha) pool_free(s->lz_alpha);
  if (s->lz_beta) pool_free(s->lz_beta);
  if (s->hc) pool_host_ctrl_free(s->hc);
  if (s->up.host) pool_host_chunk_free(s->up.host);
  if (s->lz_graph) (void)hipGraphExecDestroy(s->lz_graph);
  for (int k = 0; k < 2; k++) {
    if (s->snap[k]) pool_host_ctrl_free(s->snap[k]);
    if (s->snap_ev[k]) pool_event_free(s->snap_ev[k]);
    if (s->graph_exec[k]) (void)hipGraphExecDestroy(s->graph_exec[k]);
  }
  for (int k = 2; k < 5; k++)
    if (s->graph_exec[k]) (void)hipGraphExecDestroy(s->graph_exec[k]);
  if (s->stream) { (void)hipStreamSynchronize(s->stream); pool_stream_free(s->stream); }
  delete s;
  return SDPLR_OK;
}

int32_t sdplr_hip_reset_rank(S* s, int64_t new_r) {
  ApiShared api_guard(dev_of(s));
  NEED_FINAL_RW(s);
  if (new_r < 1 || s->n * new_r >= (1LL << 40)) return fail(s, SDPLR_ERR_INVALID_ARG, "reset_rank: bad rank");
  HIPCK(s, hipStreamSynchronize(s->stream));
  if (s->arena.base) pool_free(s->arena.base);
  s->arena.base = nullptr;
  for (int k = 0; k < 5; k++)
    if (s->graph_exec[k]) { (void)hipGraphExecDestroy(s->graph_exec[k]); s->graph_exec[k] = nullptr; }
  for (double** p : {&s->lr_part, &s->lr_W, &s->lr_WS, &s->scratchF[0], &s->scratchF[1]}) { dfree(s, *p); *p = nullptr; }
  s->r = new_r;
  int rc = SDPLR_OK;
  if (s->fast) {
    s->tiles_deferred = s->rs_ok && tiles_can_wait(s);
    if (!s->tiles_deferred) rc = build_tiles(s);
  }
  if (rc) return rc;
  if ((rc = alloc_factors(s))) return rc;
  const int64_t m = s->m;
  HIPCK(s, hipMemsetAsync(s->lambda, 0, std::max<int64_t>(m, 1) * sizeof(double), s->stream));
  HIPCK(s, hipMemsetAsync(s->pv, 0, std::max<int64_t>(m, 1) * sizeof(double), s->stream));
  for (double* p : {s->y, s->pv_raw, s->A_RD, s->A_DD}) HIPCK(s, hipMemsetAsync(p, 0, (m + 1) * sizeof(double), s->stream));
  if ((rc = dzero(s, &s->lr_part, (size_t)std::max(s->nb_lr, SDPLR_MAXNB) * 2 * std::max(s->lr.ST, 1) * s->r))) return rc;
  if ((rc = dzero(s, &s->lr_W, (size_t)2 * std::max(s->lr.ST, 1) * s->r))) return rc;
  if ((rc = dzero(s, &s->lr_WS, (size_t)std::max(s->lr.ST, 1) * s->r))) return rc;
  if ((rc = pull(s))) return rc;
  DevCtrl keep = *s->hc;
  memset(s->hc, 0, sizeof(DevCtrl));
  s->hc->sigma = keep.sigma;
  s->hc->alpha_max = 1.0;
  s->hc->latest = (int)s->h;
  s->gram_dirty = s->sg_stale = s->ynext_pending = false;
  s->P_valid = false;
  s->S_stale = false;
  return push(s);
}

int32_t sdplr_hip_set_factor(S* s, int32_t slot, const double* h) {
  ApiShared api_guard(dev_of(s));
  NEED_FINAL(s);
  s->G_consistent = false;
  { const int rc_r = ensure_canonical(s); if (rc_r) return rc_r; }
  { const int rc_d = ensure_dirt(s); if (rc_d) return rc_d; }
  double* p = factor_ptr(s, slot);
  if (!p || !h) return fail(s, SDPLR_ERR_INVALID_ARG, "set_factor: bad slot");
  {
    const int rc = h2d_copy(s, p, h, (size_t)s->N * sizeof(double));
    if (rc) return rc;
  }
  note_factor_written(s, slot);
  return SDPLR_OK;
}
int32_t sdplr_hip_get_factor(S* s, int32_t slot, double* h) {
  ApiShared api_guard(dev_of(s));
  NEED_FINAL(s);
  if (slot != SDPLR_F_RT) {
    const int rc_d = ensure_dirt(s);
    if (rc_d) return rc_d;
  }
  double* p = factor_ptr(s, slot);
  if (!p || !h) return fail(s, SDPLR_ERR_INVALID_ARG, "get_factor: bad slot");
  HIPCK(s, hipMemcpyAsync(h, p, s->N * sizeof(double), hipMemcpyDeviceToHost, s->stream));
  HIPCK(s, hipStreamSynchronize(s->stream));
  return SDPLR_OK;
}
}

namespace {
double* vec_ptr(S* s, int32_t which, int64_t* len, bool* in_ctrl) {
  const int64_t m = s->m;
  *in_ctrl = false;
  switch (which) {
    case SDPLR_V_LAMBDA: *len = m; return s->lambda;
    case SDPLR_V_LAMBDA_UB: *len = m; return s->lambda_ub;
    case SDPLR_V_B: *len = m; return s->b;
    case SDPLR_V_Y: *len = m + 1; return s->y;
    case SDPLR_V_PV_RAW: *len = m + 1; return s->pv_raw;
    case SDPLR_V_PV_LB: *len = m; return s->pv_lb;
    case SDPLR_V_PV: *len = m; return s->pv;
    case SDPLR_V_A_RD: *len = m + 1; return s->A_RD;
    case SDPLR_V_A_DD: *len = m + 1; return s->A_DD;
    case SDPLR_V_LBFGS_RHO: *len = s->h; *in_ctrl = !s->lit; return s->lit ? s->lit_rho : s->hc->rho;
    case SDPLR_V_LBFGS_A: *len = s->h; *in_ctrl = !s->lit; return s->lit ? s->lit_a : s->hc->a;
    case SDPLR_V_UVT: *len = s->nnzT; return s->sp.UVt0;
    case SDPLR_V_TRIU_S_NZVAL: *len = s->nnzT; return s->sp.triu_nzval;
    case SDPLR_V_S_NZVAL: *len = s->nnzS; return s->sp.nzval;
    case SDPLR_V_SCRATCH:
      *len = m + 1;
      if (!s->scratchV && dzero(s, &s->scratchV, (size_t)m + 1) != SDPLR_OK) *len = -1;
      return s->scratchV;
    default: *len = -1; return nullptr;
  }
// ... 22 lines not shown
    s->S_from_y = false;
    s->S_stale = false;
  }
  return SDPLR_OK;
}
int32_t sdplr_hip_get_vec(S* s, int32_t which, double* h, int64_t len) {
  ApiShared api_guard(dev_of(s));
  NEED_FINAL(s);
  int64_t L; bool in_ctrl;
  double* p = vec_ptr(s, which, &L, &in_ctrl);
  if (L < 0 || len != L || (!h && L > 0)) return fail(s, SDPLR_ERR_INVALID_ARG, "get_vec: bad slot/length");
  if (which == SDPLR_V_S_NZVAL || which == SDPLR_V_TRIU_S_NZVAL) ensure_S(s);
  if (L == 0) return SDPLR_OK;
  if (in_ctrl) {
    int rc = pull_if_stale(s);
    if (rc) return rc;
    memcpy(h, p, L * sizeof(double));
    return SDPLR_OK;
  }
  HIPCK(s, hipMemcpyAsync(h, p, L * sizeof(double), hipMemcpyDeviceToHost, s->stream));
  HIPCK(s, hipStreamSynchronize(s->stream));
  return SDPLR_OK;
}
int32_t sdplr_hip_set_scalar(S* s, int32_t which, double v) {
  ApiShared api_guard(dev_of(s));
  NEED_FINAL(s);
  s->G_consistent = false;
  int rc = pull_if_stale(s);
  if (rc) return rc;
  if (which == SDPLR_S_SIGMA) s->hc->sigma = v;
  else if (which == SDPLR_S_OBJ) s->hc->obj = v;
  else if (which == SDPLR_S_LBFGS_LATEST) {
    if (s->h > 0 && (v < 1 || v > (double)s->h)) return fail(s, SDPLR_ERR_INVALID_ARG, "set_scalar: latest out of range");
    s->hc->latest = (int)v;
    s->gram_dirty = true;
  } else return fail(s, SDPLR_ERR_INVALID_ARG, "set_scalar: bad slot");
  return push(s);
}
int32_t sdplr_hip_get_scalar(S* s, int32_t which, double* v) {
  ApiShared api_guard(dev_of(s));
  NEED_FINAL(s);
  if (!v) return fail(s, SDPLR_ERR_INVALID_ARG, "get_scalar: null");
  int rc = pull_if_stale(s);
  if (rc) return rc;
  if (which == SDPLR_S_SIGMA) *v = s->hc->sigma;
  else if (which == SDPLR_S_OBJ) *v = s->hc->obj;
  else if (which == SDPLR_S_LBFGS_LATEST) *v = (double)s->hc->latest;
  else return fail(s, SDPLR_ERR_INVALID_ARG, "get_scalar: bad slot");
  return SDPLR_OK;
}
int32_t sdplr_hip_get_dims(const S* s, int64_t* n, int64_t* m, int64_t* r, int64_t* h, int64_t* nnzT,
                           int64_t* nnzS, int64_t* nnzAgg) {
  if (!s) return SDPLR_ERR_INVALID_ARG;
  if (n) *n = s->n;
  if (m) *m = s->m;
  if (r) *r = s->r;
  if (h) *h = s->h;
  if (nnzT) *nnzT = s->nnzT;
  if (nnzS) *nnzS = s->nnzS;
  if (nnzAgg) *nnzAgg = s->nnzAgg;
  return SDPLR_OK;
}
}

namespace {

#define LV_CASE(L, V, CALL) if (s->LPR == L && s->VEC == V) { constexpr int LPR = L, VEC = V; CALL; } else
#define LV_DISPATCH(CALL)                                                                              \
  LV_CASE(1, 1, CALL) LV_CASE(2, 1, CALL) LV_CASE(4, 1, CALL) LV_CASE(8, 1, CALL) LV_CASE(16, 1, CALL) \
  LV_CASE(32, 1, CALL) LV_CASE(64, 1, CALL) LV_CASE(1, 2, CALL) LV_CASE(2, 2, CALL) LV_CASE(4, 2, CALL) \
  LV_CASE(8, 2, CALL) LV_CASE(16, 2, CALL) LV_CASE(32, 2, CALL) LV_CASE(64, 2, CALL) {}
#define TLV_CASE(L, V, CALL) if (s->tile_lpr == L && s->VEC == V) { constexpr int LPR = L, VEC = V; CALL; } else
#define TLV_DISPATCH(CALL)                                                                                \
  TLV_CASE(1, 1, CALL) TLV_CASE(2, 1, CALL) TLV_CASE(4, 1, CALL) TLV_CASE(8, 1, CALL) TLV_CASE(16, 1, CALL) \
  TLV_CASE(32, 1, CALL) TLV_CASE(64, 1, CALL) TLV_CASE(1, 2, CALL) TLV_CASE(2, 2, CALL) TLV_CASE(4, 2, CALL) \
  TLV_CASE(8, 2, CALL) TLV_CASE(16, 2, CALL) TLV_CASE(32, 2, CALL) TLV_CASE(64, 2, CALL) {}
#define RING_DISPATCH(CALL)                                                                            \
  LV_CASE(4, 2, CALL) LV_CASE(8, 2, CALL) LV_CASE(16, 2, CALL) LV_CASE(32, 2, CALL) LV_CASE(64, 2, CALL) {}
#define HM_DISPATCH(CALL)                                       \
  if (s->HM == 4) { constexpr int HM = 4; CALL; }               \
  else if (s->HM == 8) { constexpr int HM = 8; CALL; }          \
  else { constexpr int HM = 16; CALL; }

int tile_lds_attr(S* s) {
  if (s->tiles_deferred) {
    s->tiles_deferred = false;
    int rc = build_tiles(s);
    if (rc) return rc;
  }
  if (!s->use_tile || s->tile_attr_done) return SDPLR_OK;
  const int bytes = (int)(((size_t)SDPLR_NT * s->VEC * (s->tile.K + 1) + (size_t)(SDPLR_NT / s->tile_lpr) * (2 * s->tile.K + 8) + (size_t)(SDPLR_NT / 64) * 2 * s->tile_lpr * s->VEC) * sizeof(double));
  static std::mutex mu;
  std::lock_guard<std::mutex> g(mu);
  hipError_t e = hipSuccess;
#define TILE_ATTR(LRN, UNI)                                                                                                      \
  TLV_DISPATCH(({                                                                                                                  \
    static int cur_max = 0;                                                                                                       \
    if (bytes > cur_max) {                                                                                                        \
      e = hipFuncSetAttribute(reinterpret_cast<const void*>(&k_spmm_tile<LPR, VEC, LRN, UNI>), hipFuncAttributeMaxDynamicSharedMemorySize, bytes); \
      if (e == hipSuccess) cur_max = bytes;                                                                                       \
    }                                                                                                                             \
  }))
  TILE_ATTR(0, false)
  if (e == hipSuccess) { TILE_ATTR(1, false) }
  if (e == hipSuccess) { TILE_ATTR(0, true) }
  if (e == hipSuccess) { TILE_ATTR(1, true) }
#undef TILE_ATTR
  if (e != hipSuccess) return fail(s, SDPLR_ERR_HIP, std::string("hipFuncSetAttribute(k_spmm_tile): ") + hipGetErrorString(e));
  s->tile_attr_done = true;
  return SDPLR_OK;
}

void enq_lowrank(S* s, const double* X0, const double* X1, int F, int mode, double* out0, double* out1, int chk) {
  if (s->lr.ST == 0) return;
  {
    ProfScope ps(s, "lr_project");
    if (F == 1) { LV_DISPATCH((k_lr_project<LPR, VEC, 1><<<s->nb_lr, SDPLR_NT, 0, s->stream>>>(s->lr, X0, X1, (int)s->n, (int)s->r, s->lr_part, s->ctrl, chk))) }
    else { LV_DISPATCH((k_lr_project<LPR, VEC, 2><<<s->nb_lr, SDPLR_NT, 0, s->stream>>>(s->lr, X0, X1, (int)s->n, (int)s->r, s->lr_part, s->ctrl, chk))) }
  }
  int nbf = s->nb_lr;
  if (s->nb_lr > 256) {
    ProfScope ps(s, "lr_reduce");
    const int nout = F * s->lr.ST * (int)s->r;
    k_lr_reduce<<<nout, SDPLR_NT, 0, s->stream>>>(nout, s->nb_lr, s->lr_part, s->lr_W, s->ctrl, chk);
    nbf = 0;
  }
  ProfScope ps(s, "lr_finalize");
  k_lr_finalize<<<1, 1024, 0, s->stream>>>(s->lr, (int)s->r, F, nbf, s->lr_part, s->lr_W, mode, out0, out1, s->y, s->lr_WS, s->ctrl, chk);
}

void enq_A(S* s, const double* U, const double* V, int mode, double* out0, double* out1, int chk) {
  if (!s->all_covered) {
    (void)hipMemsetAsync(out0, 0, (s->m + 1) * sizeof(double), s->stream);
    if (mode == 2) (void)hipMemsetAsync(out1, 0, (s->m + 1) * sizeof(double), s->stream);
  }
  if (s->n_sparse > 0) {
    {
      ProfScope ps(s, mode == 2 ? "sddmm_linesearch" : (mode == 1 ? "sddmm_uv" : "sddmm_uu"));
      if (mode == 0) { LV_DISPATCH((k_sddmm<LPR, VEC, 0><<<s->nb_sddmm, SDPLR_NT, 0, s->stream>>>(s->sp, U, V, (int)s->r, s->ctrl, chk))) }
      else if (mode == 1) { LV_DISPATCH((k_sddmm<LPR, VEC, 1><<<s->nb_sddmm, SDPLR_NT, 0, s->stream>>>(s->sp, U, V, (int)s->r, s->ctrl, chk))) }
      else { LV_DISPATCH((k_sddmm<LPR, VEC, 2><<<s->nb_sddmm, SDPLR_NT, 0, s->stream>>>(s->sp, U, V, (int)s->r, s->ctrl, chk))) }
    }
    const int nb = s->sp.n_short_blocks + s->sp.n_chunks;
    if (nb > 0) {
      ProfScope ps(s, "segreduce");
      if (mode == 2) k_segreduce<true><<<nb, SDPLR_NT, 0, s->stream>>>(s->sp, out0, out1, s->ctrl, chk);
      else k_segreduce<false><<<nb, SDPLR_NT, 0, s->stream>>>(s->sp, out0, out1, s->ctrl, chk);
    }
    if (s->sp.n_long > 0) {
      ProfScope ps(s, "seg_finalize");
      const int nbf = (s->sp.n_long * 64 + SDPLR_NT - 1) / SDPLR_NT;
      if (mode == 2) k_seg_finalize<true><<<nbf, SDPLR_NT, 0, s->stream>>>(s->sp, out0, out1, s->ctrl, chk);
      else k_seg_finalize<false><<<nbf, SDPLR_NT, 0, s->stream>>>(s->sp, out0, out1, s->ctrl, chk);
    }
  }
  if (mode == 0) enq_lowrank(s, U, U, 1, 0, out0, out1, chk);
  else enq_lowrank(s, U, V, 2, mode, out0, out1, chk);
}

void enq_At_preprocess(S* s, int chk) {
  s->S_from_y = true;
  if (s->n_sparse <= 0) return;
  {
    ProfScope ps(s, "assemble_triu");
    k_assemble_triu<<<s->nb_nnzT, SDPLR_NT, 0, s->stream>>>(s->sp, s->y, s->ctrl, chk);
  }
// ... 245 lines not shown
  double *R = aslot(s->arena, AS_R), *G = aslot(s->arena, AS_G), *D = aslot(s->arena, AS_D);
  double *P = fast_P(s), *W = fast_W(s);
  const bool upd_fused = step_fuses_update(s);
  s->gram_nb = upd_fused ? s->nb_step : s->nb_upd;
  enq_lbfgs_dir(s, 1, 1, 1, upd_fused && !s->dot_descent);
  if (!s->all_covered) {
    (void)hipMemsetAsync(s->A_RD, 0, (s->m + 1) * sizeof(double), s->stream);
    (void)hipMemsetAsync(s->A_DD, 0, (s->m + 1) * sizeof(double), s->stream);
  }
  const bool tiled = s->use_tile && s->tile_lpr == tile_shape_lpr(s) && s->n * s->r * 8 < (1LL << 32) && s->spg.n_long_rows == 0;
  if (tiled) {
    ProfScope ps(s, "spmm_W");
    const size_t lds = ((size_t)SDPLR_NT * s->VEC * (s->tile.K + 1) + (size_t)(SDPLR_NT / s->tile_lpr) * (2 * s->tile.K + 8)) * sizeof(double);
    if (s->tile.gdiag) { TLV_DISPATCH((k_spmm_tile<LPR, VEC, 0, true><<<s->nb_tile, SDPLR_NT, lds, s->stream>>>(s->tile, (int)s->n, (int)s->m, s->ff, R, D, P, W, (int)s->r, s->lambda, s->pv_raw, s->sp_fast.UVt0, s->sp_fast.UVt1, s->partials, s->ctrl, 1, s->lr, s->lr_part, 1))) }
    else { TLV_DISPATCH((k_spmm_tile<LPR, VEC, 0><<<s->nb_tile, SDPLR_NT, lds, s->stream>>>(s->tile, (int)s->n, (int)s->m, s->ff, R, D, P, W, (int)s->r, s->lambda, s->pv_raw, s->sp_fast.UVt0, s->sp_fast.UVt1, s->partials, s->ctrl, 1, s->lr, s->lr_part, 1))) }
  } else {
  {
    ProfScope ps(s, "rowdots");
    LV_DISPATCH((k_rowdots<LPR, VEC><<<s->nb_spmm, SDPLR_NT, 0, s->stream>>>(s->sp_fast, s->ff, R, D, P, (int)s->r, SLOT_PD, s->partials, s->ctrl, 1)))
  }
  {
    ProfScope ps(s, "spmm_W");
    DevLowRank none{};
    if (s->spg.n_long_rows > 0) {
      const int nbl = std::min(s->spg.n_long_rows, 256);
      LV_DISPATCH((k_spmm_both<LPR, VEC><<<s->nb_spmm + nbl, SDPLR_NT, 0, s->stream>>>(s->spg, D, W, (int)s->r, 1.0, none, nullptr, SLOT_DW, s->partials, s->ctrl, 1, D, nbl)))
    } else {
      LV_DISPATCH((k_spmm<LPR, VEC><<<s->nb_spmm, SDPLR_NT, 0, s->stream>>>(s->spg, D, W, (int)s->r, 1.0, none, nullptr, SLOT_DW, s->partials, s->ctrl, 1, D)))
    }
  }
  }
  {
    const int nb = s->sp_fast.n_short_blocks + s->sp_fast.n_chunks;
    if (nb > 0) {
      ProfScope ps(s, "segreduce");
      k_segreduce<true><<<nb, SDPLR_NT, 0, s->stream>>>(s->sp_fast, s->A_RD, s->A_DD, s->ctrl, 1);
    }
    if (s->sp_fast.n_long > 0) {
      ProfScope ps(s, "seg_finalize");
      const int nbf = (s->sp_fast.n_long * 64 + SDPLR_NT - 1) / SDPLR_NT;
      k_seg_finalize<true><<<nbf, SDPLR_NT, 0, s->stream>>>(s->sp_fast, s->A_RD, s->A_DD, s->ctrl, 1);
    }
  }
  {
    ProfScope ps(s, "fast_fill");
    if (tiled) k_fast_fill<<<1, SDPLR_NT, 0, s->stream>>>(s->ff, s->A_RD, s->A_DD, SLOT_PD, s->nb_tile, SLOT_DW, s->nb_tile, s->partials, s->ctrl, 1);
    else k_fast_fill<<<1, SDPLR_NT, 0, s->stream>>>(s->ff, s->A_RD, s->A_DD, SLOT_PD, s->nb_spmm, SLOT_DW, s->nb_spmm + std::min(s->spg.n_long_rows, 256), s->partials, s->ctrl, 1);
  }
  enq_lowrank(s, R, D, 2, 2, s->A_RD, s->A_DD, 1);
  if (armijo) {
    {
      ProfScope ps(s, "armijo_partials");
      k_armijo_partials<<<s->nb_m, SDPLR_NT, 0, s->stream>>>(s->ctrl, (int)s->m, s->lambda, s->lambda_ub, s->pv_raw, s->A_RD, s->A_DD, s->y, s->partials, 1);
    }
    ProfScope ps(s, "armijo_pick");
    k_armijo_pick<<<1, SDPLR_NT, 0, s->stream>>>(s->ctrl, (int)s->m, s->nb_m, s->A_RD, s->A_DD, s->partials, 1, 1);
  } else {
    {
      ProfScope ps(s, "ls_partials");
      k_ls_partials<<<s->nb_m, SDPLR_NT, 0, s->stream>>>(s->ctrl, (int)s->m, s->lambda, s->pv_raw, s->A_RD, s->A_DD, s->partials, 1);
    }
    ProfScope ps(s, "ls_solve");
    k_ls_solve<<<1, SDPLR_NT, 0, s->stream>>>(s->ctrl, (int)s->m, s->nb_m, s->A_RD, s->A_DD, s->partials, 1, 1);
  }
  {
    ProfScope ps(s, "ls_commit");
    k_ls_commit<<<s->nb_m, SDPLR_NT, 0, s->stream>>>(s->ctrl, (int)s->m, s->pv_raw, s->A_RD, s->A_DD, s->pv_lb, s->pv, 1, s->y, s->lambda, s->lambda_ub, s->partials, 1, 1, s->nb_step);
  }
  if (s->lr.ST > 0) {
    ProfScope ps(s, "fast_lr_ws");
    k_fast_lr_ws<<<1, SDPLR_NT, 0, s->stream>>>(s->lr, (int)s->r, s->lr_W, s->y, s->lr_WS, s->ctrl, 1);
  }
  {
    ProfScope ps(s, "fast_step");
    if (upd_fused) {
      LV_DISPATCH((k_fast_step2<LPR, VEC, 4, false><<<s->nb_step, SDPLR_NT, 5 * 4 * SDPLR_NT * sizeof(double), s->stream>>>((int)s->n, (int)s->m, s->ff, R, D, P, W, G, (int)s->r, s->y, s->lambda, s->lambda_ub, s->pv_raw, s->pv_lb, s->pv, s->A_RD, s->A_DD, s->lr, s->lr_WS, s->partials, s->ctrl, 1, s->arena, (int)s->h, s->dot_descent ? 0 : 1)))
    } else {
      LV_DISPATCH((k_fast_step2<LPR, VEC, 0, false><<<s->nb_step, SDPLR_NT, 0, s->stream>>>((int)s->n, (int)s->m, s->ff, R, D, P, W, G, (int)s->r, s->y, s->lambda, s->lambda_ub, s->pv_raw, s->pv_lb, s->pv, s->A_RD, s->A_DD, s->lr, s->lr_WS, s->partials, s->ctrl, 1, s->arena, (int)s->h, 0)))
    }
  }
  if (!upd_fused) enq_lbfgs_update(s, 1);
}

void enq_iteration_fast2(S* s) {
  double *R = aslot(s->arena, AS_R), *G = aslot(s->arena, AS_G), *D = aslot(s->arena, AS_D);
  double *P = fast_P(s), *W = fast_W(s);
  bool lr_fused = false;
  const bool upd_fused = step_fuses_update(s);
  s->gram_nb = upd_fused ? s->nb_step : s->nb_upd;
  if (s->ring_now && s->pdrop_now) {
    enq_dir_ring(s);
    {
      ProfScope ps(s, "spmm_W");
      const size_t lds = ((size_t)SDPLR_NT * s->VEC * (s->tile.K + 1) + (size_t)(SDPLR_NT / s->tile_lpr) * (2 * s->tile.K + 8)) * sizeof(double);
      if (s->tile.gdiag) { TLV_DISPATCH((k_spmm_tile<LPR, VEC, 0, true><<<s->nb_tile, SDPLR_NT, lds, s->stream>>>(s->tile, (int)s->n, (int)s->m, s->ff, R, D, P, W, (int)s->r, s->lambda, s->pv_raw, s->A_RD, s->A_DD, s->partials, s->ctrl, 1, s->lr, s->lr_part, 0, 1, s->arena))) }
      else { TLV_DISPATCH((k_spmm_tile<LPR, VEC, 0><<<s->nb_tile, SDPLR_NT, lds, s->stream>>>(s->tile, (int)s->n, (int)s->m, s->ff, R, D, P, W, (int)s->r, s->lambda, s->pv_raw, s->A_RD, s->A_DD, s->partials, s->ctrl, 1, s->lr, s->lr_part, 0, 1, s->arena))) }
    }
    ProfScope ps(s, "fast_step");
    RING_DISPATCH((k_fast_step_ring<LPR, VEC, 4><<<s->nb_step, SDPLR_NT, 5 * 4 * SDPLR_NT * sizeof(double), s->stream>>>((int)s->n, (int)s->m, s->ff, R, W, (int)s->r, s->y, s->lambda, s->lambda_ub, s->pv_raw, s->pv_lb, s->pv, s->A_RD, s->A_DD, s->partials, s->ctrl, 1, s->arena, (int)s->h, s->nb_tile)))
    return;
  }
  const bool ring_pb = s->ring_now;
  if (ring_pb) enq_dir_ring(s);
  else
  enq_lbfgs_dir(s, 1, 1, 1, upd_fused && !s->dot_descent);
#ifdef SDPLR_PROBE_TILE_HIST
  s->ff.probe_hist[0] = G;
  for (int l = 0; l < 3; l++) {
    s->ff.probe_hist[1 + l] = aslot(s->arena, AS_S0 + std::min<int>(l, (int)s->h - 1));
    s->ff.probe_hist[4 + l] = aslot(s->arena, as_y0(s->arena) + std::min<int>(l, (int)s->h - 1));
  }
#endif
  {
    ProfScope ps(s, "spmm_W");
    if (s->use_tile && s->tile_lpr == tile_shape_lpr(s) && s->n * s->r * 8 < (1LL << 32)) {
      lr_fused = s->lr.ST == 1 && s->r <= (int64_t)s->tile_lpr * s->VEC && !s->no_lrfuse;
      const size_t lds = ((size_t)SDPLR_NT * s->VEC * (s->tile.K + 1) + (size_t)(SDPLR_NT / s->tile_lpr) * (2 * s->tile.K + 8) + (lr_fused ? (size_t)(SDPLR_NT / 64) * 2 * s->tile_lpr * s->VEC : 0)) * sizeof(double);
      if (lr_fused && s->tile.gdiag) { TLV_DISPATCH((k_spmm_tile<LPR, VEC, 1, true><<<s->nb_tile, SDPLR_NT, lds, s->stream>>>(s->tile, (int)s->n, (int)s->m, s->ff, R, D, P, W, (int)s->r, s->lambda, s->pv_raw, s->A_RD, s->A_DD, s->partials, s->ctrl, 1, s->lr, s->lr_part, 0, ring_pb ? 1 : 0, s->arena))) }
      else if (lr_fused) { TLV_DISPATCH((k_spmm_tile<LPR, VEC, 1><<<s->nb_tile, SDPLR_NT, lds, s->stream>>>(s->tile, (int)s->n, (int)s->m, s->ff, R, D, P, W, (int)s->r, s->lambda, s->pv_raw, s->A_RD, s->A_DD, s->partials, s->ctrl, 1, s->lr, s->lr_part, 0, ring_pb ? 1 : 0, s->arena))) }
      else if (s->tile_panels && s->VEC == 2 && s->tile_lpr == 16 && s->LPR == 16 && !s->tile.gdiag) {
        const size_t lds1 = ((size_t)SDPLR_NT * 1 * (s->tile.K + 1) + (size_t)(SDPLR_NT / s->LPR) * (2 * s->tile.K + 8)) * sizeof(double);
        k_spmm_tile<16, 1, 0><<<s->nb_tile, SDPLR_NT, lds1, s->stream>>>(s->tile, (int)s->n, (int)s->m, s->ff, R, D, P, W, (int)s->r, s->lambda, s->pv_raw, s->A_RD, s->A_DD, s->partials, s->ctrl, 1, s->lr, s->lr_part, 0);
      }
      else if (s->tile.gdiag) { TLV_DISPATCH((k_spmm_tile<LPR, VEC, 0, true><<<s->nb_tile, SDPLR_NT, lds, s->stream>>>(s->tile, (int)s->n, (int)s->m, s->ff, R, D, P, W, (int)s->r, s->lambda, s->pv_raw, s->A_RD, s->A_DD, s->partials, s->ctrl, 1, s->lr, s->lr_part, 0, ring_pb ? 1 : 0, s->arena))) }
      else { TLV_DISPATCH((k_spmm_tile<LPR, VEC, 0><<<s->nb_tile, SDPLR_NT, lds, s->stream>>>(s->tile, (int)s->n, (int)s->m, s->ff, R, D, P, W, (int)s->r, s->lambda, s->pv_raw, s->A_RD, s->A_DD, s->partials, s->ctrl, 1, s->lr, s->lr_part, 0, ring_pb ? 1 : 0, s->arena))) }
    } else {
      LV_DISPATCH((k_spmm_fast<LPR, VEC><<<s->nb_spmm, SDPLR_NT, 0, s->stream>>>(s->spg, (int)s->m, s->ff, R, D, P, W, (int)s->r, s->lambda, s->pv_raw, s->A_RD, s->A_DD, s->partials, s->ctrl, 1)))
    }
  }
  if (lr_fused) {
    ProfScope ps(s, "lr_reduce");
    const int nout = 2 * s->lr.ST * (int)s->r;
    k_lr_reduce<<<nout, SDPLR_NT, 0, s->stream>>>(nout, s->nb_tile, s->lr_part, s->lr_W, s->ctrl, 1);
  } else {
    enq_lowrank(s, R, D, 2, 2, s->A_RD, s->A_DD, 1);
  }
  const int nb_ls = (s->use_tile && s->tile_lpr == tile_shape_lpr(s) && s->n * s->r * 8 < (1LL << 32)) ? s->nb_tile : s->nb_spmm;
  const bool lsh = upd_fused && s->pdrop_now && s->n_extra == 1 && s->lr.ST == 0 && nb_ls <= 4 * SDPLR_NT && !s->no_lshead;
  if (!lsh) {
    ProfScope ps(s, "ls_solve_fast");
    k_ls_solve_fast<<<1, SDPLR_LSF_NT, 0, s->stream>>>(s->ctrl, (int)s->m, s->ff.gid_g, s->n_extra, s->extra_slots, (s->use_tile && s->tile_lpr == tile_shape_lpr(s) && s->n * s->r * 8 < (1LL << 32)) ? s->nb_tile : s->nb_spmm, s->A_RD, s->A_DD, s->lambda, s->lambda_ub, s->pv_raw, s->pv_lb, s->pv, s->y, s->lr.ST, (int)s->r, s->lr.col_gid, s->lr.Dcat, s->lr_W, s->lr_WS, s->partials, 1, lr_fused ? 1 : 0, s->lr.n_lr, s->lr.mat_ptr, s->lr.mat_gid, nullptr, s->extra_head);
  }
  {
    ProfScope ps(s, "fast_step");
    if (lsh) {
      LV_DISPATCH((k_fast_step2<LPR, VEC, 4, true, true, true><<<s->nb_step, SDPLR_NT, 5 * 4 * SDPLR_NT * sizeof(double), s->stream>>>((int)s->n, (int)s->m, s->ff, R, D, P, W, G, (int)s->r, s->y, s->lambda, s->lambda_ub, s->pv_raw, s->pv_lb, s->pv, s->A_RD, s->A_DD, s->lr, s->lr_WS, s->partials, s->ctrl, 1, s->arena, (int)s->h, 1, nb_ls)))
    } else if (upd_fused && s->pdrop_now) {
      LV_DISPATCH((k_fast_step2<LPR, VEC, 4, true, true><<<s->nb_step, SDPLR_NT, 5 * 4 * SDPLR_NT * sizeof(double), s->stream>>>((int)s->n, (int)s->m, s->ff, R, D, P, W, G, (int)s->r, s->y, s->lambda, s->lambda_ub, s->pv_raw, s->pv_lb, s->pv, s->A_RD, s->A_DD, s->lr, s->lr_WS, s->partials, s->ctrl, 1, s->arena, (int)s->h, 1)))
    } else if (ring_pb) {
      RING_DISPATCH((k_fast_step_ring<LPR, VEC, 4, true><<<s->nb_step, SDPLR_NT, 5 * 4 * SDPLR_NT * sizeof(double), s->stream>>>((int)s->n, (int)s->m, s->ff, R, W, (int)s->r, s->y, s->lambda, s->lambda_ub, s->pv_raw, s->pv_lb, s->pv, s->A_RD, s->A_DD, s->partials, s->ctrl, 1, s->arena, (int)s->h, 0, P, s->lr, s->lr_WS)))
    } else if (upd_fused) {
      LV_DISPATCH((k_fast_step2<LPR, VEC, 4, true><<<s->nb_step, SDPLR_NT, 5 * 4 * SDPLR_NT * sizeof(double), s->stream>>>((int)s->n, (int)s->m, s->ff, R, D, P, W, G, (int)s->r, s->y, s->lambda, s->lambda_ub, s->pv_raw, s->pv_lb, s->pv, s->A_RD, s->A_DD, s->lr, s->lr_WS, s->partials, s->ctrl, 1, s->arena, (int)s->h, s->dot_descent ? 0 : 1)))
    } else {
      LV_DISPATCH((k_fast_step2<LPR, VEC, 0, true><<<s->nb_step, SDPLR_NT, 0, s->stream>>>((int)s->n, (int)s->m, s->ff, R, D, P, W, G, (int)s->r, s->y, s->lambda, s->lambda_ub, s->pv_raw, s->pv_lb, s->pv, s->A_RD, s->A_DD, s->lr, s->lr_WS, s->partials, s->ctrl, 1, s->arena, (int)s->h, 0)))
    }
  }
  if (!upd_fused) enq_lbfgs_update(s, 1);
}

double wall_clock_hz() {
  static const double hz = [] {
    int dev = 0, khz = 0;
    (void)hipGetDevice(&dev);
    if (hipDeviceGetAttribute(&khz, hipDeviceAttributeWallClockRate, dev) != hipSuccess || khz <= 0) khz = 100000;
    return 1e3 * (double)khz;
  }();
  return hz;
}
bool rs_loop_applies(const S* s, int armijo) {
  if (!s->rs_ok || armijo || s->h < 1 || s->h > 4 || s->prof_on) return false;
  if (s->force_graph || getenv("SDPLR_HIP_NO_RESIDENT") != nullptr) return false;
  return rs_loop_lds(s) <= RS_LDS_MAX;
}
bool rs_lanczos_ell_applies(const S* s) {
  if (!s->rs_ok || !s->S_from_y || s->prof_on) return false;
  if (s->force_graph || getenv("SDPLR_HIP_NO_RESIDENT") != nullptr || getenv("SDPLR_HIP_CLASSIC_LANCZOS") != nullptr) return false;
  return (size_t)4 * s->n * sizeof(double) <= RS_LDS_MAX;
}
bool rs_fg_applies(const S* s) {
  if (!s->rs_ok || s->prof_on) return false;
  if (s->force_graph || getenv("SDPLR_HIP_NO_RESIDENT") != nullptr) return false;
// ... 386 lines not shown
  if (use_graph) {
    for (int64_t k = 0; k < rounds; k += reps) { HIPCK(s, hipGraphLaunch(s->lz_graph, s->stream)); s->st_lz_graph++; }
  } else {
    for (int64_t k = 0; k < rounds; k++) three();
    s->st_lz_eager += rounds;
  }
  HIPCK(s, hipGetLastError());
  HIPCK(s, hipMemcpyAsync(alpha, s->lz_alpha, q * sizeof(double), hipMemcpyDeviceToHost, s->stream));
  HIPCK(s, hipMemcpyAsync(beta, s->lz_beta, q * sizeof(double), hipMemcpyDeviceToHost, s->stream));
  if ((rc = pull(s))) return rc;
  *steps = s->hc->lz_steps;
  return SDPLR_OK;
}

}

extern "C" {

int32_t sdplr_hip_A(S* s, int32_t u_slot, int32_t v_slot, int32_t out_vec) {
  ApiShared api_guard(dev_of(s));
  NEED_FINAL_RW(s);
  double* U = factor_ptr(s, u_slot);
  double* V = v_slot >= 0 ? factor_ptr(s, v_slot) : nullptr;
  if (!U || (v_slot >= 0 && !V)) return fail(s, SDPLR_ERR_INVALID_ARG, "A: bad factor slot");
  double* out = out_vec == SDPLR_V_PV_RAW ? s->pv_raw : out_vec == SDPLR_V_A_RD ? s->A_RD : out_vec == SDPLR_V_A_DD ? s->A_DD : nullptr;
  if (out_vec == SDPLR_V_SCRATCH) {
    int64_t L; bool in_ctrl;
    out = vec_ptr(s, SDPLR_V_SCRATCH, &L, &in_ctrl);
  }
  if (!out) return fail(s, SDPLR_ERR_INVALID_ARG, "A: bad output vector");
  enq_A(s, U, V, V ? 1 : 0, out, nullptr, 0);
  return sync_check(s);
}
int32_t sdplr_hip_At_preprocess(S* s) {
  ApiShared api_guard(dev_of(s));
  NEED_FINAL_RW(s);
  enq_At_preprocess(s, 0);
  s->S_stale = false;
  return sync_check(s);
}
int32_t sdplr_hip_At_left(S* s, int32_t ys, int32_t xs) {
  ApiShared api_guard(dev_of(s));
  NEED_FINAL_RW(s);
  double *Y = factor_ptr(s, ys), *X = factor_ptr(s, xs);
  if (!Y || !X || Y == X) return fail(s, SDPLR_ERR_INVALID_ARG, "At_left: bad slots");
  ensure_S(s);
  enq_At_left(s, Y, X, 1.0, -1, 0);
  note_factor_written(s, ys);
  return sync_check(s);
}
int32_t sdplr_hip_At_right(S* s, const double* x, double* yh, int64_t k) {
  ApiShared api_guard(dev_of(s));
  NEED_FINAL_RW(s);
  if (!x || !yh || k < 1) return fail(s, SDPLR_ERR_INVALID_ARG, "At_right: bad args");
  ensure_S(s);
  const int64_t n = s->n;
  for (int64_t c = 0; c < k; c++) {
    HIPCK(s, hipMemcpyAsync(s->lz_buf[0], x + c * n, n * sizeof(double), hipMemcpyHostToDevice, s->stream));
    enq_spmv(s, s->lz_buf[0], s->lz_buf[1], -1, nullptr);
    HIPCK(s, hipMemcpyAsync(yh + c * n, s->lz_buf[1], n * sizeof(double), hipMemcpyDeviceToHost, s->stream));
    HIPCK(s, hipStreamSynchronize(s->stream));
  }
  return sync_check(s);
}

int32_t sdplr_hip_At_right_device(S* s, const double* x, double* yd, int64_t k) {
  ApiShared api_guard(dev_of(s));
  NEED_FINAL_RW(s);
  if (!x || !yd || k < 1 || x == yd) return fail(s, SDPLR_ERR_INVALID_ARG, "At_right_device: bad args");
  hipPointerAttribute_t ax{}, ay{};
  if (hipPointerGetAttributes(&ax, x) != hipSuccess || hipPointerGetAttributes(&ay, yd) != hipSuccess ||
      ax.type != hipMemoryTypeDevice || ay.type != hipMemoryTypeDevice) {
    (void)hipGetLastError();
    return fail(s, SDPLR_ERR_INVALID_ARG, "At_right_device: x and y must be device pointers");
  }
  ensure_S(s);
  const int64_t n = s->n;
  for (int64_t c = 0; c < k; c++) enq_spmv(s, x + c * n, yd + c * n, -1, nullptr);
  return sync_check(s);
}

int32_t sdplr_hip_get_stats(const S* s, int64_t* out, int32_t cap, int32_t* n_written) {
  if (!s || !out || cap < 0) return SDPLR_ERR_INVALID_ARG;
  const int64_t v[16] = {s->st_captures, s->st_capture_failed, s->st_capture_skipped, s->st_graph_batches,
                         s->st_eager_batches, s->st_lz_graph, s->st_lz_eager, s->st_iters, s->st_rs_loops, s->st_rs_lz, s->st_rs_fg,
                         s->st_rs_shared, s->st_pdrop, s->st_grp_loops, s->st_ring_loops, s->st_ring_materialized};
  const int32_t k = std::min<int32_t>(cap, 16);
  for (int32_t i = 0; i < k; i++) out[i] = v[i];
  if (n_written) *n_written = k;
  return SDPLR_OK;
}

int32_t sdplr_hip_f(S* s, double* L) {
  ApiShared api_guard(dev_of(s));
  NEED_FINAL_RW(s);
  enq_f(s);
  int rc = pull(s);
  if (rc) return rc;
  if (L) *L = s->hc->L;
  return sync_check(s);
}
int32_t sdplr_hip_g(S* s) {
  ApiShared api_guard(dev_of(s));
  NEED_FINAL_RW(s);
  enq_g(s, 0, false);
  s->S_stale = false;
  s->sg_stale = true;
  s->G_consistent = true;
  s->G_age = 0;
  return sync_check(s);
}
}

namespace {
RsFgArgs rs_fg_args(S* s) {
  RsFgArgs a{};
  a.lr = rs_lr(s);
  a.rowvec = rs_rows_global(s) ? s->rs_rowvec : nullptr;
  a.n = (int)s->n; a.m = (int)s->m; a.r = (int)s->r;
  a.gid_g = s->ff.gid_g; a.row_k = s->rs_row_k; a.row_v = s->rs_row_v; a.E = s->rs_ell;
  a.R = aslot(s->arena, AS_R); a.G = aslot(s->arena, AS_G); a.P = aslot(s->arena, 3 + 2 * (int)s->h);
  a.y = s->y; a.pv_raw = s->pv_raw; a.pv = s->pv;
  a.lam = s->lambda; a.lam_ub = s->lambda_ub; a.lb = s->pv_lb; a.b = s->b;
  a.c = s->ctrl;
  return a;
}
int set_norm_params(S* s, double normC, double normb, int grel, int prel) {
  int rc = pull(s);
  if (rc) return rc;
  s->hc->normC = normC; s->hc->normb = normb; s->hc->grel = grel; s->hc->prel = prel;
  s->hc->done = 0; s->hc->err = 0;
  return push(s);
}
}

extern "C" {
int32_t sdplr_hip_fg(S* s, double normC, double normb, int32_t grel, int32_t prel, double* L, double* gn, double* pn) {
  ApiShared api_guard(dev_of(s));
  NEED_FINAL_RW(s);
  int rc = set_norm_params(s, normC, normb, grel, prel);
  if (rc) return rc;
  if (rs_fg_applies(s)) {
    const RsFgArgs a = rs_fg_args(s);
    const size_t lds = rs_loop_lds(s);
    RS_VEC_DISPATCH(s, ({ RS_SET_ATTR((k_rs_fg<VEC>)); k_rs_fg<VEC><<<1, SDPLR_RS_NT, lds, s->stream>>>(a); }))
    HIPCK(s, hipGetLastError());
    s->P_valid = true;
    s->P_age = 0;
    s->S_stale = true;
    s->S_from_y = true;
    s->sg_stale = true;
    s->G_consistent = true;
    s->G_age = 0;
    s->st_rs_fg++;
    if ((rc = pull(s))) return rc;
    if (L) *L = s->hc->L;
    if (gn) *gn = s->hc->gnorm;
    if (pn) *pn = s->hc->pvnorm;
    return sync_check(s);
  }
  if (s->fast && s->fast_singleton && s->lr.ST == 0 && s->use_tile && !s->tiles_deferred && s->tile_lpr == tile_shape_lpr(s) &&
      s->n * s->r * 8 < (1LL << 32) && getenv("SDPLR_HIP_NO_FAST_FG") == nullptr) {
    if ((rc = tile_lds_attr(s))) return rc;
    double *R = aslot(s->arena, AS_R), *G = aslot(s->arena, AS_G), *P = fast_P(s);
    if (!s->all_covered) HIPCK(s, hipMemsetAsync(s->A_DD, 0, (s->m + 1) * sizeof(double), s->stream));
    {
      ProfScope ps(s, "spmm_P");
      const size_t lds = ((size_t)SDPLR_NT * s->VEC * (s->tile.K + 1) + (size_t)(SDPLR_NT / s->tile_lpr) * (2 * s->tile.K + 8)) * sizeof(double);
      if (s->tile.gdiag) { TLV_DISPATCH((k_spmm_tile<LPR, VEC, 0, true><<<s->nb_tile, SDPLR_NT, lds, s->stream>>>(s->tile, (int)s->n, (int)s->m, s->ff, R, R, P, P, (int)s->r, s->lambda, s->pv_raw, s->A_RD, s->A_DD, s->partials, s->ctrl, 0, s->lr, s->lr_part, 0))) }
      else { TLV_DISPATCH((k_spmm_tile<LPR, VEC, 0><<<s->nb_tile, SDPLR_NT, lds, s->stream>>>(s->tile, (int)s->n, (int)s->m, s->ff, R, R, P, P, (int)s->r, s->lambda, s->pv_raw, s->A_RD, s->A_DD, s->partials, s->ctrl, 0, s->lr, s->lr_part, 0))) }
// ... 187 lines not shown
  return inner_loop_impl(s, normC, normb, grel, prel, use_armijo, cur_gtol, fprec_eps, max_local_iters, time_budget_s, Lio, gnio,
                         pnio, last_alpha, iters, exit_reason, false);
}
static int32_t inner_loop_impl(S* s, double normC, double normb, int32_t grel, int32_t prel, int32_t use_armijo,
                               double cur_gtol, double fprec_eps, int64_t max_local_iters, double time_budget_s,
                               double* Lio, double* gnio, double* pnio, double* last_alpha, int64_t* iters,
                               int32_t* exit_reason, bool resume) {
  ApiLock api_lock(g_api_rw);
  bind_device(dev_of(s));
  const bool hc_was_valid = s && s->finalized && s->hc_valid;
  const bool G_was_consistent = s && s->finalized && s->G_consistent;
  const int dirt_was_from = (s && s->finalized) ? s->dirt_from : -1;
  bool ring_keep = false;
  if (s && s->finalized && s->ring_on) {
    const bool fast2_ = s->fast && s->fast_singleton && !use_armijo;
    static const int64_t refresh_iters_ = getenv("SDPLR_HIP_P_REFRESH_ITERS") ? atoll(getenv("SDPLR_HIP_P_REFRESH_ITERS")) : 256;
    const bool would_pdrop = fast2_ && step_can_drop_P(s) && s->G_consistent && (!resume || s->pdrop_now);
    const bool refresh_due = would_pdrop && !resume && s->G_age >= refresh_iters_;
    ring_keep = fast2_ && ring_shape_common(s) && !refresh_due && !s->ring_unc && Lio && gnio && pnio &&
                max_local_iters >= 1 && !rs_loop_applies(s, use_armijo) &&
                !(s->gram_dirty || s->ynext_pending || s->sg_stale);
    if (ring_keep) s->ring_on = false;
  }
  if (s && s->finalized && max_local_iters >= 1 && Lio && gnio && pnio) s->dirt_from = -1;
  NEED_FINAL_RW(s);
  if (ring_keep) s->ring_on = true;
  if (!Lio || !gnio || !pnio || max_local_iters < 1) return fail(s, SDPLR_ERR_INVALID_ARG, "inner_loop: bad args");
  const bool gram_work = s->h > 0 && (s->gram_dirty || s->ynext_pending || s->sg_stale);
  ensure_gram(s);
  int rc = rs_loop_applies(s, use_armijo) ? SDPLR_OK : tile_lds_attr(s);
  if (rc) return rc;
  s->hc_valid = hc_was_valid && !gram_work;
  if ((rc = pull_if_stale(s))) return rc;
  s->hc_valid = false;
  DevCtrl* c = s->hc;
  c->done = 0; c->exit_reason = 0; c->err = 0; c->use_armijo = use_armijo;
  c->iters = 0; c->max_iters = max_local_iters; c->reldelta_exit = 0; c->norms_pending = 0; c->pv2_extra = 0.0;
  c->cur_gtol = cur_gtol; c->fprec_eps = fprec_eps; c->normC = normC; c->normb = normb;
  c->grel = grel; c->prel = prel;
  c->L = *Lio; c->gnorm = *gnio; c->pvnorm = *pnio; c->alpha = 0.0; c->alpha_max = 1.0;
  HIPCK(s, hipMemcpyAsync(s->ctrl, s->hc, sizeof(DevCtrl), hipMemcpyHostToDevice, s->stream));
  if (rs_loop_applies(s, use_armijo)) {
    s->dirt_from = dirt_was_from;
    if ((rc = ensure_dirt(s))) return rc;
    return run_resident_loop(s, time_budget_s, false, false, Lio, gnio, pnio, last_alpha, iters, exit_reason, nullptr, G_was_consistent, resume);
  }
  const bool fastp = s->fast;
  const bool fast2 = fastp && s->fast_singleton && !use_armijo;
  static const int64_t refresh_iters = getenv("SDPLR_HIP_P_REFRESH_ITERS") ? atoll(getenv("SDPLR_HIP_P_REFRESH_ITERS")) : 256;
  s->pdrop_now = fast2 && step_can_drop_P(s) && G_was_consistent && (!resume || s->pdrop_now);
  if (s->pdrop_now && !resume && s->G_age >= refresh_iters) {
    enq_g(s, 0, false);
    s->S_stale = false;
    s->G_age = 0;
  }
  s->ring_now = fast2 && (s->pdrop_now ? ring_shape_ok(s) : ring_shape_pb_ok(s));
  if (getenv("SDPLR_HIP_DEBUG"))
    fprintf(stderr, "[sdplr_hip] inner_loop: ring %d (kept %d, pdrop %d, shape %d: can_drop %d n_extra %d VEC %d LPR %d tile %d/%d nb_tile %d)\n",
            (int)s->ring_now, (int)ring_keep, (int)s->pdrop_now, (int)ring_shape_ok(s), (int)step_can_drop_P(s), s->n_extra,
            s->VEC, s->LPR, (int)s->use_tile, s->tile_lpr, s->nb_tile);
  if (s->ring_on && !s->ring_now) {
    if ((rc = ensure_canonical(s))) return rc;
  }
  {
    const bool fresh = s->ring_now && !s->ring_on;
    const int was = c->ring_on;
    if (fresh) {
      c->ring_k = 0; c->ring_n = 0; c->ring_unc = 0;
      c->ring_j0 = c->latest % (int)s->h;
      memset(c->ring_alpha, 0, sizeof c->ring_alpha);
    }
    c->ring_on = s->ring_now ? 1 : 0;
    if (fresh || was != c->ring_on)
      HIPCK(s, hipMemcpyAsync(&s->ctrl->ring_on, &c->ring_on, sizeof(DevCtrl) - offsetof(DevCtrl, ring_on), hipMemcpyHostToDevice, s->stream));
    s->ring_on = s->ring_now;
  }
  auto bail = [&](int rc_) {
    s->ring_on = false;
    s->gram_dirty = true;
    s->G_consistent = false;
    s->hc_valid = false;
    return rc_;
  };
  const int ar = use_armijo ? 1 : (s->ring_now ? (s->pdrop_now ? 3 : 4) : (s->pdrop_now ? 2 : 0));
  const bool edgep = !fastp && edge_applies(s, use_armijo);
  auto enq_iter = [&]() {
    if (fast2) enq_iteration_fast2(s);
    else if (fastp) enq_iteration_fast(s, use_armijo);
    else if (edgep) enq_iteration_edge(s);
    else enq_iteration(s, use_armijo);
  };
  if (fastp || edgep) { s->S_stale = true; s->S_from_y = true; }
  if (s->pdrop_now) {
    s->P_valid = false;
  } else if (fastp) {
    if (!s->P_valid || (!resume && s->P_age >= refresh_iters)) {
      enq_fast_refresh_P(s);
      s->P_valid = true;
      s->P_age = 0;
    }
  }
  bool use_graph = !s->prof_on && !s->graph_disabled && max_local_iters >= 4 && getenv("SDPLR_HIP_NO_GRAPH") == nullptr &&
                   (s->N >= (1LL << 17) || s->force_graph);
  if (use_graph && !s->graph_exec[ar]) {
    api_lock.unlock();
    {
      std::unique_lock<ApiMutex> excl(g_api_rw, std::chrono::milliseconds(capture_wait_ms()));
      if (!excl.owns_lock()) {
        s->st_capture_skipped++;
      } else {
        hipGraph_t graph = nullptr;
        bool ok = hipStreamBeginCapture(s->stream, hipStreamCaptureModeRelaxed) == hipSuccess;
        if (ok) {
          for (int i = 0; i < s->graph_iters; i++) enq_iter();
          ok = hipStreamEndCapture(s->stream, &graph) == hipSuccess && graph != nullptr;
        }
        if (ok) ok = hipGraphInstantiate(&s->graph_exec[ar], graph, nullptr, nullptr, 0) == hipSuccess;
        if (graph) (void)hipGraphDestroy(graph);
        if (ok) {
          s->st_captures++;
        } else {
          note_capture_failure(s, "inner loop");
          s->graph_exec[ar] = nullptr;
        }
      }
    }
    api_lock.lock();
  }
  if (!s->graph_exec[ar]) use_graph = false;
  const auto t0 = std::chrono::steady_clock::now();
  const int64_t eager_batch = 8;
  int64_t planned = 0;
  bool plan_closed = false;
  const bool dbg = getenv("SDPLR_HIP_DEBUG") != nullptr;
  double t_enq = 0.0, t_wait = 0.0;
  int n_batches = 0;
  auto now = [] { return std::chrono::duration<double>(std::chrono::steady_clock::now().time_since_epoch()).count(); };
  auto launch_batch = [&](int slot) -> int {
    const double ta = now();
    n_batches++;
    const int64_t left = max_local_iters - planned;
    if (use_graph && left >= s->graph_iters) {
      HIPCK(s, hipGraphLaunch(s->graph_exec[ar], s->stream));
      planned += s->graph_iters;
      s->st_graph_batches++;
    } else if (left > 0) {
      const int64_t nb_it = std::min<int64_t>(left, eager_batch);
      for (int64_t i = 0; i < nb_it; i++) enq_iter();
      HIPCK(s, hipGetLastError());
      planned += nb_it;
      s->st_eager_batches++;
    }
    if (planned >= max_local_iters && !plan_closed) {
      const bool lf = fastp ? step_fuses_update(s) : spmm_fuses_update(s);
      s->gram_nb = !lf ? s->nb_upd : (fastp ? s->nb_step : spmm_upd_blocks(s));
      enq_boundary(s, 0, 1, 1, 0);
      plan_closed = true;
    }
    HIPCK(s, hipMemcpyAsync(s->snap[slot], s->ctrl, sizeof(DevCtrl), hipMemcpyDeviceToHost, s->stream));
    HIPCK(s, hipEventRecord(s->snap_ev[slot], s->stream));
    t_enq += now() - ta;
    return SDPLR_OK;
  };
  int why = -1;
  int final_snap = -1;
  if (s->prof_on) {
    int64_t passes = 0;
    for (;;) {
      const int64_t nb = std::min<int64_t>(8, max_local_iters - passes);
      for (int64_t i = 0; i < nb; i++) enq_iter();
      passes += std::max<int64_t>(nb, 0);
      if (nb <= 0) {
        s->prof_on = false;
        enq_iter();
        s->prof_on = true;
      }
      if (hipError_t e_ = hipGetLastError(); e_ != hipSuccess) return bail(fail(s, SDPLR_ERR_HIP, std::string("inner_loop: ") + hipGetErrorString(e_)));
      if ((rc = pull(s))) return bail(rc);
      if (c->done) break;
      if (time_budget_s > 0 &&
          std::chrono::duration<double>(std::chrono::steady_clock::now() - t0).count() > time_budget_s) {
        why = EXIT_TIME;
        break;
      }
    }
  } else {
    int cur = 0;
    if ((rc = launch_batch(cur))) return bail(rc);
    for (;;) {
      const bool more = !plan_closed;
      if (more && (rc = launch_batch(cur ^ 1))) return bail(rc);
      const double tw = now();
      if (hipError_t e_ = hipEventSynchronize(s->snap_ev[cur]); e_ != hipSuccess) return bail(fail(s, SDPLR_ERR_HIP, std::string("inner_loop: ") + hipGetErrorString(e_)));
      t_wait += now() - tw;
      if (s->snap[cur]->done) {
        if (!more && plan_closed) final_snap = cur;
        break;
      }
      if (time_budget_s > 0) {
        const double el = std::chrono::duration<double>(std::chrono::steady_clock::now() - t0).count();
        if (el > time_budget_s) { why = EXIT_TIME; break; }
      }
      if (!more) break;
      cur ^= 1;
    }
  }
  const bool loop_fused = fastp ? step_fuses_update(s) : spmm_fuses_update(s);
  s->gram_nb = !loop_fused ? s->nb_upd : (fastp ? s->nb_step : spmm_upd_blocks(s));
  if (fastp || edgep) { s->S_stale = true; s->S_from_y = true; }
  if (final_snap >= 0) {
    memcpy(s->hc, s->snap[final_snap], sizeof(DevCtrl));
    s->hc_valid = true;
  } else {
    enq_boundary(s, 0, 1, 0, 0);
    if ((rc = pull(s))) return bail(rc);
  }
  if (s->ring_now) {
    s->ring_k = c->ring_k; s->ring_n = c->ring_n; s->ring_unc = c->ring_unc; s->ring_latest = c->latest; s->ring_j0 = c->ring_j0;
    memcpy(s->ring_alpha, c->ring_alpha, sizeof s->ring_alpha);
  }
  if (c->done) why = c->exit_reason;
  if (loop_fused && c->iters > 0 && c->err == 0 && why != EXIT_RELDELTA) {
    s->dirt_from = c->latest - 1;
  } else if (c->iters == 0 && c->err == 0) {
    s->dirt_from = dirt_was_from;
  }
  if (dbg)
    fprintf(stderr, "[sdplr_hip] inner_loop: %d batches (%s), host enqueue %.3f ms, host wait %.3f ms, iters %lld\n",
            n_batches, use_graph ? "graph" : "eager", 1e3 * t_enq, 1e3 * t_wait, (long long)c->iters);
  s->sg_stale = (why == EXIT_RELDELTA);
  s->ynext_pending = (why == EXIT_RELDELTA) && s->h > 0;
  if (c->err == SDPLR_ERR_NOT_DESCENT) {
    const int latest_ = c->latest;
    c->err = 0; c->done = 0;
    (void)push(s);
    if (s->ring_now) { s->st_ring_loops++; s->ring_unc = 2; }
    s->P_age += c->iters;
    s->G_age = s->pdrop_now ? s->G_age + c->iters : 0;
    if ((rc = park_ynext_after_not_descent(s, latest_))) return rc;
    return fail(s, SDPLR_ERR_NOT_DESCENT, "Error: cubic[1] should be less than 0.");
  }
  s->st_iters += c->iters;
  s->P_age += c->iters;
  s->G_age = s->pdrop_now ? s->G_age + c->iters : 0;
  if (s->pdrop_now) s->st_pdrop++;
  if (s->ring_now) s->st_ring_loops++;
  s->G_consistent = true;
  *Lio = c->L; *gnio = c->gnorm; *pnio = c->pvnorm;
  if (last_alpha) *last_alpha = c->alpha;
  if (iters) *iters = c->iters;
  if (exit_reason) *exit_reason = why;
  return sync_check(s);
}

int32_t sdplr_hip_major_iteration(S* s, double normC, double normb, int32_t grel, int32_t prel, int32_t use_armijo,
                                  int32_t update_lambda, double sigma, double cur_gtol, double fprec_eps,
                                  int64_t max_local_iters, double time_budget_s, double* L, double* gn, double* pn,
                                  double* last_alpha, int64_t* iters, int32_t* exit_reason) {
  if (!s) return fail(nullptr, SDPLR_ERR_INVALID_ARG, "null handle");
  if (!L || !gn || !pn || max_local_iters < 1) return fail(s, SDPLR_ERR_INVALID_ARG, "major_iteration: bad args");
  if (update_lambda == SDPLR_MAJOR_RESUME)
    return inner_loop_impl(s, normC, normb, grel, prel, use_armijo, cur_gtol, fprec_eps, max_local_iters, time_budget_s, L, gn, pn,
                           last_alpha, iters, exit_reason, true);
  bool resident = false;
  {
    ApiShared api_guard(dev_of(s));
    { const int rc_r = ring_drop_for_clear(s); if (rc_r) return rc_r; }
    NEED_FINAL_RW(s);
    resident = rs_loop_applies(s, use_armijo) && rs_fg_applies(s);
    if (resident) {
      RsLoopIn in{};
      in.sigma = sigma; in.gtol = cur_gtol; in.fprec = fprec_eps; in.normC = normC; in.normb = normb;
      in.grel = grel; in.prel = prel; in.max_iters = max_local_iters;
      s->sg_stale = s->ynext_pending = false;
      return run_resident_loop(s, time_budget_s, update_lambda != 0, true, L, gn, pn, last_alpha, iters, exit_reason, &in);
    }
  }
  int32_t rc;
  if (update_lambda && (rc = sdplr_hip_update_lambda(s))) return rc;
  if ((rc = sdplr_hip_set_scalar(s, SDPLR_S_SIGMA, sigma))) return rc;
  if ((rc = sdplr_hip_lbfgs_clear(s))) return rc;
  if ((rc = sdplr_hip_fg(s, normC, normb, grel, prel, L, gn, pn))) return rc;
  if (last_alpha) *last_alpha = 0.0;
  if (iters) *iters = 0;
  if (exit_reason) *exit_reason = EXIT_GTOL;
  if (!(*gn > cur_gtol)) return SDPLR_OK;
  return sdplr_hip_inner_loop(s, normC, normb, grel, prel, use_armijo, cur_gtol, fprec_eps, max_local_iters, time_budget_s,
                              L, gn, pn, last_alpha, iters, exit_reason);
}

int32_t sdplr_hip_lanczos(S* s, int64_t q, const double* v0, double* alpha, double* beta, int64_t* steps) {
  ApiShared api_guard(dev_of(s));
  NEED_FINAL_RW_KEEP_HISTORY(s);
  if (!v0 || !alpha || !beta || !steps || q < 1) return fail(s, SDPLR_ERR_INVALID_ARG, "lanczos: bad args");
  ensure_S(s);
  return run_lanczos(s, q, v0, alpha, beta, steps, &api_guard.l);
}
int32_t sdplr_hip_tridiag_mineig(const double* alpha, const double* beta, int64_t k, double* out) {
  if (!alpha || !out || k < 1 || (k > 1 && !beta)) return SDPLR_ERR_INVALID_ARG;
  if (k == 1) { *out = (alpha[0] + 1) - 1; return SDPLR_OK; }
  std::vector<double> d(k);
  for (int64_t i = 0; i < k; i++) d[i] = alpha[i] + 1;
  double lo = std::numeric_limits<double>::infinity(), hi = -lo;
  for (int64_t i = 0; i < k; i++) {
    const double rad = (i > 0 ? std::fabs(beta[i - 1]) : 0.0) + (i + 1 < k ? std::fabs(beta[i]) : 0.0);
    lo = std::min(lo, d[i] - rad);
    hi = std::max(hi, d[i] + rad);
  }
  for (int it = 0; it < 200; it++) {
    const double mid = 0.5 * (lo + hi);
    if (mid <= lo || mid >= hi) break;
    if (sturm_below(d, beta, k, mid) >= 1) hi = mid; else lo = mid;
  }
  *out = 0.5 * (lo + hi) - 1;
  return SDPLR_OK;
}
static int32_t approx_mineig_impl(S* s, int64_t q, const double* v0, double* mineig, ApiLock* api_lock) {
  std::vector<double> al(q), be(q);
  int64_t steps = 0;
  int rc = run_lanczos(s, q, v0, al.data(), be.data(), &steps, api_lock);
  if (rc) return rc;
  return sdplr_hip_tridiag_mineig(al.data(), be.data(), steps, mineig);
}
int32_t sdplr_hip_approx_mineigval_lanczos(S* s, int64_t q, const double* v0, double* mineig) {
  ApiShared api_guard(dev_of(s));
  NEED_FINAL_RW_KEEP_HISTORY(s);
  if (!v0 || !mineig || q < 1) return fail(s, SDPLR_ERR_INVALID_ARG, "approx_mineigval_lanczos: bad args");
  ensure_S(s);
  return approx_mineig_impl(s, q, v0, mineig, &api_guard.l);
// ... 852 lines not shown
```

Measured before the change: 6308.

## Fuse fast step, L-BFGS seam and next direction into one persistent kernel

```diff
diff --git a/sdplrplus.jl_amd/cabi.py b/sdplrplus.jl_amd/cabi.py
--- a/sdplrplus.jl_amd/cabi.py
+++ b/sdplrplus.jl_amd/cabi.py
@@ -22,7 +22,7 @@
 STAT_NAMES = ("graph_captures", "graph_capture_failures", "graph_capture_skipped", "graph_batches",
               "eager_batches", "lanczos_graph_replays", "lanczos_eager_rounds", "inner_iterations",
               "resident_loops", "resident_lanczos", "resident_fg", "resident_shared_launches", "p_less_loops",
-              "group_launch_loops", "ring_history_loops", "ring_materializations")
+              "group_launch_loops", "ring_history_loops", "ring_materializations", "fused_step_dir_loops")
 S_SIGMA, S_OBJ, S_LBFGS_LATEST = 0, 1, 2
 
 _i32, _i64, _f64, _vp = C.c_int32, C.c_int64, C.c_double, C.c_void_p
diff --git a/sdplrplus.jl_amd/csrc/k_dense.h b/sdplrplus.jl_amd/csrc/k_dense.h
--- a/sdplrplus.jl_amd/csrc/k_dense.h
+++ b/sdplrplus.jl_amd/csrc/k_dense.h
@@ -287,16 +287,22 @@
   }
 }
 
-__device__ __forceinline__ void lbfgs_boundary_body(DevCtrl* __restrict__ c, int h, int jfixed, int fin_mode, int do_loop, int do_coeff, int nb_partials, const double* __restrict__ partials, int desc_mode, double* __restrict__ pv_raw, int m) {
-  __shared__ SeamLds gd;
-  const int tid = threadIdx.x, wave = tid >> 6, lane = tid & 63;
+template <int NTHR = 1024>
+__device__ __forceinline__ void lbfgs_boundary_body(SeamLds& gd, DevCtrl* c, int h, int jfixed, int fin_mode, int do_loop, int do_coeff, int nb_partials, const double* partials, int desc_mode, double* pv_raw, int m) {
+  static_assert(NTHR % 64 == 0 && 1024 % NTHR == 0, "whole waves, a divisor of the 1024-thread layout");
+  constexpr int NWORDS = (int)(sizeof(DevCtrl) / 8);
+  constexpr int NCW = (NWORDS + NTHR - 1) / NTHR;
+  const int tid = threadIdx.x, lane = tid & 63;
 #ifdef SDPLR_STAMPS
   const unsigned long long st0 = __builtin_amdgcn_s_memtime();
 #endif
   const int gp = c->gram_pending, np = c->norms_pending;
   const int op = c->obj_pending;
   static_assert(sizeof(DevCtrl) / 8 <= 1024, "one word of the control block per thread");
-  const unsigned long long cw = reinterpret_cast<const unsigned long long*>(c)[min(tid, (int)(sizeof(DevCtrl) / 8) - 1)];
+  unsigned long long cw[NCW];
+#pragma unroll
+  for (int q = 0; q < NCW; q++) cw[q] = reinterpret_cast<const unsigned long long*>(c)[min(tid + q * NTHR, NWORDS - 1)];
+  for (int wave = tid >> 6; wave < 16; wave += NTHR / 64)
   if (wave >= 14) {
     const int nbp = (wave == 14) ? c->nb_gnorm : c->nb_pvnorm;
     const double* p = slot_partials(partials, wave == 14 ? SLOT_GNORM2 : SLOT_PVNORM2);
@@ -339,7 +345,9 @@
       }
     }
   }
-  if (tid < (int)(sizeof(DevCtrl) / 8)) reinterpret_cast<unsigned long long*>(&gd.c)[tid] = cw;
+#pragma unroll
+  for (int q = 0; q < NCW; q++)
+    if (tid + q * NTHR < NWORDS) reinterpret_cast<unsigned long long*>(&gd.c)[tid + q * NTHR] = cw[q];
   const bool fin = (fin_mode == 2) || (fin_mode == 1 && gp);
   const bool norms = np != 0;
   if (!fin && !do_coeff && !do_loop && !norms && !op) return;
@@ -377,7 +385,7 @@
   {
     const unsigned long long* src = reinterpret_cast<const unsigned long long*>(&gd.c);
     unsigned long long* dst = reinterpret_cast<unsigned long long*>(c);
-    for (int t = tid; t < (int)(sizeof(DevCtrl) / 8); t += 1024) dst[t] = src[t];
+    for (int t = tid; t < NWORDS; t += NTHR) dst[t] = src[t];
   }
 #ifdef SDPLR_STAMPS
   asm volatile("s_waitcnt vmcnt(0)" ::: "memory");
@@ -391,7 +399,8 @@
 k_lbfgs_boundary(DevCtrl* __restrict__ c, int h, int jfixed, int fin_mode, int do_loop, int do_coeff,
                  int nb_partials, const double* __restrict__ partials, int desc_mode, double* __restrict__ pv_raw = nullptr,
                  int m = 0) {
-  lbfgs_boundary_body(c, h, jfixed, fin_mode, do_loop, do_coeff, nb_partials, partials, desc_mode, pv_raw, m);
+  __shared__ SeamLds gd;
+  lbfgs_boundary_body<1024>(gd, c, h, jfixed, fin_mode, do_loop, do_coeff, nb_partials, partials, desc_mode, pv_raw, m);
 }
 
 template <int HM, bool NTH>
diff --git a/sdplrplus.jl_amd/csrc/k_group.h b/sdplrplus.jl_amd/csrc/k_group.h
--- a/sdplrplus.jl_amd/csrc/k_group.h
+++ b/sdplrplus.jl_amd/csrc/k_group.h
@@ -81,7 +81,8 @@
 
 __global__ void __launch_bounds__(1024) k_grp_boundary(const GrpSeamArgs* __restrict__ tab) {
   const GrpSeamArgs a = tab[blockIdx.y];
-  lbfgs_boundary_body(a.c, a.h, a.jfixed, a.fin_mode, a.do_loop, a.do_coeff, a.nb_partials, a.partials, a.desc_mode, a.pv_raw, a.m);
+  __shared__ SeamLds gd;
+  lbfgs_boundary_body<1024>(gd, a.c, a.h, a.jfixed, a.fin_mode, a.do_loop, a.do_coeff, a.nb_partials, a.partials, a.desc_mode, a.pv_raw, a.m);
 }
 template <int HM>
 __global__ void __launch_bounds__(SDPLR_NT) k_grp_dir(const GrpDirArgs* __restrict__ tab) {
diff --git a/sdplrplus.jl_amd/csrc/k_sparse.h b/sdplrplus.jl_amd/csrc/k_sparse.h
--- a/sdplrplus.jl_amd/csrc/k_sparse.h
+++ b/sdplrplus.jl_amd/csrc/k_sparse.h
@@ -1,4 +1,6 @@
 #pragma once
+#include <type_traits>
+
 #include "common.h"
 #include "k_dense.h"
 #include "k_scalar.h"
@@ -1032,15 +1034,70 @@
   }
 }
 
-template <int LPR, int VEC, int HMU, bool PB = false>
-__global__ void __launch_bounds__(SDPLR_NT)
-k_fast_step_ring(int n, int m, DevFast ff, double* __restrict__ R, const double* __restrict__ W, int r,
-                 double* __restrict__ yvec, const double* __restrict__ lam, const double* __restrict__ lam_ub,
-                 double* __restrict__ pv_raw, const double* __restrict__ lb, double* __restrict__ pv,
-                 const double* __restrict__ A_RD, const double* __restrict__ A_DD, double* __restrict__ partials,
-                 DevCtrl* __restrict__ c, int check_done, FactorArena A, int h, int nb_ls,
-                 double* __restrict__ P = nullptr, DevLowRank lr = DevLowRank{}, const double* __restrict__ WS = nullptr) {
+#define SDPLR_ERR_FUSED_BARRIER (-103)
+#define SDPLR_FUSE_KR 3
+#define SDPLR_GBAR_WORDS (17 * 16)
+struct GridBar {
+  unsigned long long* w;
+  long long spin_cap;
+};
+__device__ __forceinline__ bool grid_barrier(const GridBar& gb, DevCtrl* c, int* sh_ok) {
+  asm volatile("s_waitcnt vmcnt(0)" ::: "memory");
+  __syncthreads();
+  if (threadIdx.x == 0) {
+    const unsigned nb = gridDim.x, g = blockIdx.x & 7u;
+    const unsigned long long cnt = (nb - g + 7u) >> 3, ng = nb < 8u ? nb : 8u;
+    unsigned long long* sub = gb.w + 16 * g;
+    unsigned long long* top = gb.w + 16 * 8;
+    unsigned long long* gen = gb.w + 16 * (9 + g);
+    __builtin_amdgcn_fence(__ATOMIC_RELEASE, "agent");
+    const unsigned long long old = __hip_atomic_fetch_add(sub, 1ull, __ATOMIC_RELAXED, __HIP_MEMORY_SCOPE_AGENT);
+    const unsigned long long round = old / cnt + 1;
+    const long long t0 = wall_clock64();
+    int ok = 1;
+    if ((old + 1) % cnt == 0) {
+      __builtin_amdgcn_fence(__ATOMIC_ACQUIRE, "agent");
+      __builtin_amdgcn_fence(__ATOMIC_RELEASE, "agent");
+      const unsigned long long told = __hip_atomic_fetch_add(top, 1ull, __ATOMIC_RELAXED, __HIP_MEMORY_SCOPE_AGENT);
+      const unsigned long long target = (told / ng + 1) * ng;
+      while (__hip_atomic_load(top, __ATOMIC_RELAXED, __HIP_MEMORY_SCOPE_AGENT) < target) {
+        if (wall_clock64() - t0 > gb.spin_cap) { ok = 0; break; }
+        __builtin_amdgcn_s_sleep(2);
+      }
+      __builtin_amdgcn_fence(__ATOMIC_ACQUIRE, "agent");
+      if (ok) __hip_atomic_store(gen, round, __ATOMIC_RELEASE, __HIP_MEMORY_SCOPE_AGENT);
+    } else {
+      while (__hip_atomic_load(gen, __ATOMIC_RELAXED, __HIP_MEMORY_SCOPE_AGENT) < round) {
+        if (wall_clock64() - t0 > gb.spin_cap) { ok = 0; break; }
+        __builtin_amdgcn_s_sleep(2);
+      }
+    }
+    if (!ok) {
+      __hip_atomic_store(&c->err, SDPLR_ERR_FUSED_BARRIER, __ATOMIC_RELAXED, __HIP_MEMORY_SCOPE_AGENT);
+      __hip_atomic_store(&c->done, 1, __ATOMIC_RELAXED, __HIP_MEMORY_SCOPE_AGENT);
+    }
+    *sh_ok = ok;
+  }
+  __syncthreads();
+  const int ok = *sh_ok;
+  __builtin_amdgcn_fence(__ATOMIC_ACQUIRE, "agent");
+  return ok != 0;
+}
+__device__ __forceinline__ double ld_agent(const double* p) {
+  return __longlong_as_double((long long)__hip_atomic_load(reinterpret_cast<const unsigned long long*>(p), __ATOMIC_RELAXED, __HIP_MEMORY_SCOPE_AGENT));
+}
+__device__ __forceinline__ int ld_agent(const int* p) { return __hip_atomic_load(p, __ATOMIC_RELAXED, __HIP_MEMORY_SCOPE_AGENT); }
+
+template <int LPR, int VEC, int HMU, bool PB, bool FUSE>
+__device__ __forceinline__ void
+fast_step_ring_body(int n, int m, DevFast ff, double* __restrict__ R, const double* __restrict__ W, int r,
+                    double* __restrict__ yvec, const double* __restrict__ lam, const double* __restrict__ lam_ub,
+                    double* __restrict__ pv_raw, const double* __restrict__ lb, double* __restrict__ pv,
+                    const double* __restrict__ A_RD, const double* __restrict__ A_DD, double* __restrict__ partials,
+                    DevCtrl* __restrict__ c, int check_done, FactorArena A, int h, int nb_ls,
+                    double* __restrict__ P, DevLowRank lr, const double* __restrict__ WS, GridBar gb, int nth) {
   static_assert(HMU >= 1, "the ring form rides the fused update");
+  static_assert(!FUSE || (!PB && HMU == 4 && VEC == 2), "the fused form: P-less, the direction kernel's HM = 4");
   __shared__ double sh[2 * (SDPLR_NT / 64)];
   __shared__ double shl[10 * (SDPLR_NT / 64)];
   extern __shared__ double accl[];
@@ -1153,7 +1210,12 @@
   for (int k = 0; k < 5 * HMU; k++) accl[k * SDPLR_NT + threadIdx.x] = 0.0;
   constexpr int TR = LPR < SDPLR_STEP_TR ? LPR : SDPLR_STEP_TR;
   const long long ntiles = ((long long)n + TR - 1) / TR;
-  for (long long tile = (long long)blockIdx.x * G + threadIdx.x / LPR; tile < ntiles; tile += total) {
+  constexpr int KR = FUSE ? SDPLR_FUSE_KR : 1;
+  static_assert(!FUSE || SDPLR_FUSE_KR + 1 >= TR, "the first trip is kept whole");
+  vecd<VEC> kg[KR][1 + HMU], kd[KR][1 + HO];
+  double* const keepl = accl + 5 * HMU * SDPLR_NT + threadIdx.x;
+  auto trip = [&](const long long tile, auto first_tag) __attribute__((always_inline)) {
+    constexpr bool FIRST = decltype(first_tag)::value;
     const long long j0 = tile * TR;
     const int nrows = (int)min((long long)TR, (long long)n - j0);
     if (dn) return;
@@ -1180,7 +1242,7 @@
         pv_raw[k] = v;
       }
     }
-    for (int i0 = 0; i0 < nrows; i0 += 2) {
+    auto rowpair = [&](const int i0) __attribute__((always_inline)) {
       vecd<VEC> xx[2], pq[2], dd[2], ww[2], gv[2][HMU], dv[2][HO];
       double dj[2], dq[2];
       unsigned off[2];
@@ -1260,6 +1322,27 @@
 #else
         strow<VEC>(rowat(Gnew, off[u]), g);
 #endif
+        if constexpr (FUSE && FIRST) {
+          const int ri = i0 + u;
+          if (ri < KR) {
+            kg[ri][0] = g;
+            kd[ri][0] = d;
+#pragma unroll
+            for (int l = 0; l < HMU; l++) kg[ri][1 + l] = gv[u][l];
+#pragma unroll
+            for (int l = 0; l < HO; l++) kd[ri][1 + l] = dv[u][l];
+          } else {
+#pragma unroll
+            for (int q = 0; q < VEC; q++) {
+              keepl[(0 * VEC + q) * SDPLR_NT] = g.v[q];
+              keepl[((1 + HMU) * VEC + q) * SDPLR_NT] = d.v[q];
+#pragma unroll
+              for (int l = 0; l < HMU; l++) keepl[((1 + l) * VEC + q) * SDPLR_NT] = gv[u][l].v[q];
+#pragma unroll
+              for (int l = 0; l < HO; l++) keepl[((2 + HMU + l) * VEC + q) * SDPLR_NT] = dv[u][l].v[q];
+            }
+          }
+        }
         if (upd) {
           vecd<VEC> sn, yn;
 #pragma unroll
@@ -1307,7 +1390,25 @@
           }
         }
       }
-    }
+    };
+    if constexpr (FIRST) {
+#pragma unroll
+      for (int i0 = 0; i0 < TR; i0 += 2)
+        if (i0 < nrows) rowpair(i0);
+    } else {
+      for (int i0 = 0; i0 < nrows; i0 += 2) rowpair(i0);
+    }
+  };
+  const long long tile0 = (long long)blockIdx.x * G + threadIdx.x / LPR;
+  {
+    long long tile = tile0;
+    if constexpr (FUSE) {
+      if (tile < ntiles) {
+        trip(tile, std::true_type{});
+        tile += total;
+      }
+    }
+    for (; tile < ntiles; tile += total) trip(tile, std::false_type{});
   }
   if (dn) return;
   __syncthreads();
@@ -1333,6 +1434,149 @@
       c->nb_pvnorm = gridDim.x;
     }
   }
+  if constexpr (FUSE) {
+    __shared__ int sh_ok;
+    if (!grid_barrier(gb, c, &sh_ok)) return;
+    static_assert(sizeof(SeamLds) <= 5 * HMU * SDPLR_NT * sizeof(double), "the seam's LDS fits the Gram columns");
+    if (blockIdx.x == 0) lbfgs_boundary_body<SDPLR_NT>(*reinterpret_cast<SeamLds*>(accl), c, h, 0, 1, 1, 1, (int)gridDim.x, partials, 1, pv_raw, m);
+    if (!grid_barrier(gb, c, &sh_ok)) return;
+    if (ld_agent(&c->done)) return;
+    const int latest2 = ld_agent(&c->latest), rk2 = ld_agent(&c->ring_k), rn2 = ld_agent(&c->ring_n), fb = ld_agent(&c->fallback);
+    constexpr int HM = HMU;
+    double ca[HM], cg[HM], ra2[HM];
+    int slot[HM];
+    {
+      int j = latest2 - 1;
+#pragma unroll
+      for (int i = 0; i < HM; i++) {
+        const int jj = (i < h && j >= 0) ? j : 0;
+        slot[i] = jj;
+        const double a0 = ld_agent(&c->c_alpha[jj]), g0 = ld_agent(&c->c_gamma[jj]), r0 = ld_agent(&c->ring_alpha[jj]);
+        ca[i] = (i < h) ? a0 : 0.0;
+        cg[i] = (i < h) ? g0 : 0.0;
+        ra2[i] = (i < rn2) ? r0 : 1.0;
+        j = (j <= 0) ? h - 1 : j - 1;
+      }
+    }
+    auto direction = [&](const vecd<VEC> (&gq)[HM + 1], const vecd<VEC> (&dq)[HM]) {
+      vecd<VEC> d;
+#pragma unroll
+      for (int q = 0; q < VEC; q++) {
+        double rr = gq[0].v[q];
+#pragma unroll
+        for (int k = 0; k < HM; k++) {
+          const bool ring = k < rn2;
+          const double yx = ring ? gq[k].v[q] - gq[k + 1].v[q] : gq[k + 1].v[q];
+          rr -= ca[k] * yx;
+        }
+#pragma unroll
+        for (int k = HM - 1; k >= 0; k--) {
+          const double sx = ra2[k] * dq[k].v[q];
+          rr += cg[k] * sx;
+        }
+        d.v[q] = -1.0 * rr;
+        if (fb) d.v[q] = -gq[0].v[q];
+      }
+      return d;
+    };
+    double* const dir = ring_D(A, rk2, rj0);
+    if (ch0 >= r) return;
+    long long tile = tile0;
+    if (tile < ntiles) {
+      const long long j0 = tile * TR;
+      const int nrows = (int)min((long long)TR, (long long)n - j0);
+#pragma unroll
+      for (int ri = 0; ri < TR; ri++) {
+        if (ri >= nrows) break;
+        vecd<VEC> gq[HM + 1], dq[HM];
+        if (ri < KR) {
+#pragma unroll
+          for (int l = 0; l <= HM; l++) gq[l] = kg[ri][l];
+#pragma unroll
+          for (int l = 0; l < HM; l++) dq[l] = kd[ri][l];
+        } else {
+#pragma unroll
+          for (int q = 0; q < VEC; q++) {
+#pragma unroll
+            for (int l = 0; l <= HM; l++) gq[l].v[q] = keepl[(l * VEC + q) * SDPLR_NT];
+#pragma unroll
+            for (int l = 0; l < HM; l++) dq[l].v[q] = keepl[((1 + HMU + l) * VEC + q) * SDPLR_NT];
+          }
+        }
+#pragma unroll
+        for (int k = 0; k < HM; k++)
+          if (k >= h) gq[k + 1] = dq[k] = gq[0];
+        const unsigned off = (unsigned)(((unsigned long long)(j0 + ri) * (unsigned)r + (unsigned)ch0) * 8ull);
+        strow<VEC>(rowat(dir, off), direction(gq, dq));
+      }
+      tile += total;
+    }
+    if (tile >= ntiles) return;
+    const double* gp2[HM + 1];
+    const double* dp2[HM];
+    gp2[0] = ring_G(A, rk2, rj0);
+#pragma unroll
+    for (int i = 0; i < HM; i++) {
+      if (i >= h) {
+        gp2[i + 1] = gp2[0];
+        dp2[i] = gp2[0];
+      } else if (i < rn2) {
+        gp2[i + 1] = ring_G(A, ring_back(rk2, i + 1, h), rj0);
+        dp2[i] = ring_D(A, ring_back(rk2, i + 1, h), rj0);
+      } else {
+        gp2[i + 1] = aslot(A, as_y0(A) + slot[i]);
+        dp2[i] = aslot(A, AS_S0 + slot[i]);
+      }
+    }
+    for (; tile < ntiles; tile += total) {
+      const long long j0 = tile * TR;
+      const int nrows = (int)min((long long)TR, (long long)n - j0);
+      for (int i0 = 0; i0 < nrows; i0 += 2) {
+        vecd<VEC> gq[2][HM + 1], dq[2][HM];
+        unsigned off[2];
+#pragma unroll
+        for (int u = 0; u < 2; u++) {
+          const int i = min(i0 + u, nrows - 1);
+          off[u] = (unsigned)(((unsigned long long)(j0 + i) * (unsigned)r + (unsigned)ch0) * 8ull);
+          gq[u][0] = ldrow_nt<VEC>(rowat(gp2[0], off[u]));
+#pragma unroll
+          for (int k = 0; k < HM; k++) {
+            if (nth) {
+              gq[u][k + 1] = ldrow_nt<VEC>(rowat(gp2[k + 1], off[u]));
+              dq[u][k] = ldrow_nt<VEC>(rowat(dp2[k], off[u]));
+            } else {
+              gq[u][k + 1] = ldrow<VEC>(rowat(gp2[k + 1], off[u]));
+              dq[u][k] = ldrow<VEC>(rowat(dp2[k], off[u]));
+            }
+          }
+        }
+#pragma unroll
+        for (int u = 0; u < 2; u++) {
+          if (i0 + u >= nrows) break;
+          strow<VEC>(rowat(dir, off[u]), direction(gq[u], dq[u]));
+        }
+      }
+    }
+  }
+}
+template <int LPR, int VEC, int HMU, bool PB = false>
+__global__ void __launch_bounds__(SDPLR_NT)
+k_fast_step_ring(int n, int m, DevFast ff, double* __restrict__ R, const double* __restrict__ W, int r,
+                 double* __restrict__ yvec, const double* __restrict__ lam, const double* __restrict__ lam_ub,
+                 double* __restrict__ pv_raw, const double* __restrict__ lb, double* __restrict__ pv,
+                 const double* __restrict__ A_RD, const double* __restrict__ A_DD, double* __restrict__ partials,
+                 DevCtrl* __restrict__ c, int check_done, FactorArena A, int h, int nb_ls,
+                 double* __restrict__ P = nullptr, DevLowRank lr = DevLowRank{}, const double* __restrict__ WS = nullptr) {
+  fast_step_ring_body<LPR, VEC, HMU, PB, false>(n, m, ff, R, W, r, yvec, lam, lam_ub, pv_raw, lb, pv, A_RD, A_DD, partials, c, check_done, A, h,
+                                                nb_ls, P, lr, WS, GridBar{}, 0);
+}
+template <int LPR, int VEC, int HMU>
+__global__ void __launch_bounds__(SDPLR_NT, 2)
+k_fast_step_dir_ring(int n, int m, DevFast ff, double* R, const double* W, int r, double* yvec, const double* lam,
+                     const double* lam_ub, double* pv_raw, const double* lb, double* pv, const double* A_RD, const double* A_DD,
+                     double* partials, DevCtrl* c, int check_done, FactorArena A, int h, int nb_ls, GridBar gb, int nth) {
+  fast_step_ring_body<LPR, VEC, HMU, false, true>(n, m, ff, R, W, r, yvec, lam, lam_ub, pv_raw, lb, pv, A_RD, A_DD, partials, c, check_done, A, h,
+                                                  nb_ls, nullptr, DevLowRank{}, nullptr, gb, nth);
 }
 
 template <int LPR, int VEC>
diff --git a/sdplrplus.jl_amd/csrc/sdplr_hip.hip b/sdplrplus.jl_amd/csrc/sdplr_hip.hip
--- a/sdplrplus.jl_amd/csrc/sdplr_hip.hip
+++ b/sdplrplus.jl_amd/csrc/sdplr_hip.hip
@@ -131,6 +131,12 @@
   bool pdrop_now = false;
   bool no_ring = false;
   bool ring_on = false, ring_now = false;
+  bool no_fused_dir = true;
+  int fused_fit = -1;
+  bool fused_token = false;
+  bool fused_now = false;
+  bool fz_skip_dir = false, fz_fuse_step = false;
+  double* fused_bar = nullptr;
   int ring_k = 0, ring_n = 0, ring_unc = 0, ring_latest = 0, ring_j0 = 0;
   double ring_alpha[SDPLR_HMAX] = {};
   bool G_consistent = false;
@@ -176,7 +182,7 @@
   int nb_upd = 1;
   int nb_dense = 1, nb_m = 1, nb_sddmm = 1, nb_spmm = 1, nb_spmv = 1, nb_nnzT = 1, nb_nnzS = 1, nb_n = 1;
 
-  hipGraphExec_t graph_exec[5] = {nullptr, nullptr, nullptr, nullptr, nullptr};
+  hipGraphExec_t graph_exec[6] = {nullptr, nullptr, nullptr, nullptr, nullptr, nullptr};
   int graph_iters = 8;
   bool graph_disabled = false;
   hipGraphExec_t lz_graph = nullptr;
@@ -190,7 +196,7 @@
   double* scratchF[2] = {nullptr, nullptr};
   double* scratchV = nullptr;
   int64_t st_captures = 0, st_capture_failed = 0, st_capture_skipped = 0, st_graph_batches = 0,
-          st_eager_batches = 0, st_lz_graph = 0, st_lz_eager = 0, st_iters = 0, st_rs_loops = 0, st_rs_lz = 0, st_rs_fg = 0, st_rs_shared = 0, st_pdrop = 0, st_grp_loops = 0, st_ring_loops = 0, st_ring_materialized = 0;
+          st_eager_batches = 0, st_lz_graph = 0, st_lz_eager = 0, st_iters = 0, st_rs_loops = 0, st_rs_lz = 0, st_rs_fg = 0, st_rs_shared = 0, st_pdrop = 0, st_grp_loops = 0, st_ring_loops = 0, st_ring_materialized = 0, st_fused_loops = 0;
 
   bool prof_on = false;
   std::string prof_filter;
@@ -205,6 +211,7 @@
 namespace {
 using S = sdplr_hip_solver;
 inline int dev_of(const S* s) { return s ? s->device : -1; }
+void fused_token_release(S* s);
 void ensure_S(S* s);
 
 int fail(S* s, int code, const std::string& msg) {
@@ -1726,6 +1733,7 @@
     s->pv_lb = const_cast<double*>(lb);
   }
   if ((rc = dzero(s, &s->partials, (size_t)SDPLR_NSLOT * SDPLR_MAXNB))) return rc;
+  if ((rc = dzero(s, &s->fused_bar, SDPLR_GBAR_WORDS))) return rc;
   for (int k = 0; k < 3; k++)
     if ((rc = dzero(s, &s->lz_buf[k], n + 64))) return rc;
   if ((rc = dzero(s, &s->lz_v0, n))) return rc;
@@ -1764,6 +1772,7 @@
   s->no_pdrop = getenv("SDPLR_HIP_NO_PDROP") != nullptr;
   s->no_lshead = getenv("SDPLR_HIP_NO_LSHEAD") != nullptr;
   s->no_ring = getenv("SDPLR_HIP_NO_RING") != nullptr;
+  s->no_fused_dir = getenv("SDPLR_HIP_NO_FUSED_DIR") != nullptr || getenv("SDPLR_HIP_FUSED_DIR") == nullptr;
   s->tile_panels = getenv("SDPLR_HIP_TILE_PANELS") != nullptr;
   if (s->have_sparse && getenv("SDPLR_HIP_NO_FAST") == nullptr) {
     std::vector<int> general;
@@ -2036,9 +2045,10 @@
     if (s->snap_ev[k]) pool_event_free(s->snap_ev[k]);
     if (s->graph_exec[k]) (void)hipGraphExecDestroy(s->graph_exec[k]);
   }
-  for (int k = 2; k < 5; k++)
+  for (int k = 2; k < 6; k++)
     if (s->graph_exec[k]) (void)hipGraphExecDestroy(s->graph_exec[k]);
   if (s->stream) { (void)hipStreamSynchronize(s->stream); pool_stream_free(s->stream); }
+  fused_token_release(s);
   delete s;
   return SDPLR_OK;
 }
@@ -2050,8 +2060,9 @@
   HIPCK(s, hipStreamSynchronize(s->stream));
   if (s->arena.base) pool_free(s->arena.base);
   s->arena.base = nullptr;
-  for (int k = 0; k < 5; k++)
+  for (int k = 0; k < 6; k++)
     if (s->graph_exec[k]) { (void)hipGraphExecDestroy(s->graph_exec[k]); s->graph_exec[k] = nullptr; }
+  s->fused_fit = -1;
   for (double** p : {&s->lr_part, &s->lr_W, &s->lr_WS, &s->scratchF[0], &s->scratchF[1]}) { dfree(s, *p); *p = nullptr; }
   s->r = new_r;
   int rc = SDPLR_OK;
@@ -2240,6 +2251,41 @@
   else if (s->HM == 8) { constexpr int HM = 8; CALL; }          \
   else { constexpr int HM = 16; CALL; }
 
+static std::mutex g_fused_mu;
+static std::map<int, const S*> g_fused_owner;
+bool fused_token_acquire(S* s) {
+  if (s->fused_token) return true;
+  std::lock_guard<std::mutex> lk(g_fused_mu);
+  auto it = g_fused_owner.find(s->device);
+  if (it != g_fused_owner.end() && it->second != nullptr) return false;
+  g_fused_owner[s->device] = s;
+  s->fused_token = true;
+  return true;
+}
+void fused_token_release(S* s) {
+  if (!s->fused_token) return;
+  std::lock_guard<std::mutex> lk(g_fused_mu);
+  g_fused_owner[s->device] = nullptr;
+  s->fused_token = false;
+}
+inline size_t fused_lds_bytes(const S* s) { return (size_t)(5 * 4 + 9 * s->VEC) * SDPLR_NT * sizeof(double); }
+int fused_fit_check(S* s) {
+  if (s->fused_fit >= 0) return SDPLR_OK;
+  s->fused_fit = 0;
+  hipError_t e = hipSuccess;
+  int per_cu = 0, cus = 0;
+  const int bytes = (int)fused_lds_bytes(s);
+  RING_DISPATCH(({
+    const void* k = reinterpret_cast<const void*>(&k_fast_step_dir_ring<LPR, VEC, 4>);
+    e = hipFuncSetAttribute(k, hipFuncAttributeMaxDynamicSharedMemorySize, bytes);
+    if (e == hipSuccess) e = hipOccupancyMaxActiveBlocksPerMultiprocessor(&per_cu, k_fast_step_dir_ring<LPR, VEC, 4>, SDPLR_NT, (size_t)bytes);
+  }))
+  if (e == hipSuccess) e = hipDeviceGetAttribute(&cus, hipDeviceAttributeMultiprocessorCount, s->device);
+  if (e != hipSuccess) return fail(s, SDPLR_ERR_HIP, std::string("fused step + direction kernel: ") + hipGetErrorString(e));
+  s->fused_fit = ((long long)per_cu * cus >= (long long)s->nb_step) ? 1 : 0;
+  return SDPLR_OK;
+}
+
 int tile_lds_attr(S* s) {
   if (s->tiles_deferred) {
     s->tiles_deferred = false;
@@ -2651,6 +2697,7 @@
   if (!upd_fused) enq_lbfgs_update(s, 1);
 }
 
+double wall_clock_hz();
 void enq_iteration_fast2(S* s) {
   double *R = aslot(s->arena, AS_R), *G = aslot(s->arena, AS_G), *D = aslot(s->arena, AS_D);
   double *P = fast_P(s), *W = fast_W(s);
@@ -2658,7 +2705,7 @@
   const bool upd_fused = step_fuses_update(s);
   s->gram_nb = upd_fused ? s->nb_step : s->nb_upd;
   if (s->ring_now && s->pdrop_now) {
-    enq_dir_ring(s);
+    if (!s->fz_skip_dir) enq_dir_ring(s);
     {
       ProfScope ps(s, "spmm_W");
       const size_t lds = ((size_t)SDPLR_NT * s->VEC * (s->tile.K + 1) + (size_t)(SDPLR_NT / s->tile_lpr) * (2 * s->tile.K + 8)) * sizeof(double);
@@ -2666,6 +2713,13 @@
       else { TLV_DISPATCH((k_spmm_tile<LPR, VEC, 0><<<s->nb_tile, SDPLR_NT, lds, s->stream>>>(s->tile, (int)s->n, (int)s->m, s->ff, R, D, P, W, (int)s->r, s->lambda, s->pv_raw, s->A_RD, s->A_DD, s->partials, s->ctrl, 1, s->lr, s->lr_part, 0, 1, s->arena))) }
     }
     ProfScope ps(s, "fast_step");
+    if (s->fz_fuse_step) {
+      static const long long nt_above = getenv("SDPLR_HIP_DIR_NT_ABOVE_MB") ? atoll(getenv("SDPLR_HIP_DIR_NT_ABOVE_MB")) << 20 : 200LL << 20;
+      const long long arena_bytes = (long long)(3 + 2 * s->h + (s->fast ? 2 : 0)) * s->arena.stride * (long long)sizeof(double);
+      const GridBar gb{reinterpret_cast<unsigned long long*>(s->fused_bar), (long long)(2.0 * wall_clock_hz())};
+      RING_DISPATCH((k_fast_step_dir_ring<LPR, VEC, 4><<<s->nb_step, SDPLR_NT, fused_lds_bytes(s), s->stream>>>((int)s->n, (int)s->m, s->ff, R, W, (int)s->r, s->y, s->lambda, s->lambda_ub, s->pv_raw, s->pv_lb, s->pv, s->A_RD, s->A_DD, s->partials, s->ctrl, 1, s->arena, (int)s->h, s->nb_tile, gb, arena_bytes > nt_above ? 1 : 0)))
+      return;
+    }
     RING_DISPATCH((k_fast_step_ring<LPR, VEC, 4><<<s->nb_step, SDPLR_NT, 5 * 4 * SDPLR_NT * sizeof(double), s->stream>>>((int)s->n, (int)s->m, s->ff, R, W, (int)s->r, s->y, s->lambda, s->lambda_ub, s->pv_raw, s->pv_lb, s->pv, s->A_RD, s->A_DD, s->partials, s->ctrl, 1, s->arena, (int)s->h, s->nb_tile)))
     return;
   }
@@ -3218,10 +3272,10 @@
 
 int32_t sdplr_hip_get_stats(const S* s, int64_t* out, int32_t cap, int32_t* n_written) {
   if (!s || !out || cap < 0) return SDPLR_ERR_INVALID_ARG;
-  const int64_t v[16] = {s->st_captures, s->st_capture_failed, s->st_capture_skipped, s->st_graph_batches,
+  const int64_t v[17] = {s->st_captures, s->st_capture_failed, s->st_capture_skipped, s->st_graph_batches,
                          s->st_eager_batches, s->st_lz_graph, s->st_lz_eager, s->st_iters, s->st_rs_loops, s->st_rs_lz, s->st_rs_fg,
-                         s->st_rs_shared, s->st_pdrop, s->st_grp_loops, s->st_ring_loops, s->st_ring_materialized};
-  const int32_t k = std::min<int32_t>(cap, 16);
+                         s->st_rs_shared, s->st_pdrop, s->st_grp_loops, s->st_ring_loops, s->st_ring_materialized, s->st_fused_loops};
+  const int32_t k = std::min<int32_t>(cap, 17);
   for (int32_t i = 0; i < k; i++) out[i] = v[i];
   if (n_written) *n_written = k;
   return SDPLR_OK;
@@ -3575,13 +3629,26 @@
     s->hc_valid = false;
     return rc_;
   };
-  const int ar = use_armijo ? 1 : (s->ring_now ? (s->pdrop_now ? 3 : 4) : (s->pdrop_now ? 2 : 0));
+  s->fused_now = false;
+  if (s->ring_now && s->pdrop_now && !s->no_fused_dir && !s->prof_on && s->h >= 1 && s->h <= 4) {
+    if ((rc = fused_fit_check(s))) return bail(rc);
+    s->fused_now = s->fused_fit == 1 && fused_token_acquire(s);
+  }
+  const int ar = use_armijo ? 1 : (s->ring_now ? (s->pdrop_now ? (s->fused_now ? 5 : 3) : 4) : (s->pdrop_now ? 2 : 0));
   const bool edgep = !fastp && edge_applies(s, use_armijo);
   auto enq_iter = [&]() {
     if (fast2) enq_iteration_fast2(s);
     else if (fastp) enq_iteration_fast(s, use_armijo);
     else if (edgep) enq_iteration_edge(s);
     else enq_iteration(s, use_armijo);
+  };
+  auto enq_iters = [&](int64_t count) {
+    for (int64_t i = 0; i < count; i++) {
+      s->fz_skip_dir = s->fused_now && i > 0;
+      s->fz_fuse_step = s->fused_now && i + 1 < count;
+      enq_iter();
+    }
+    s->fz_skip_dir = s->fz_fuse_step = false;
   };
   if (fastp || edgep) { s->S_stale = true; s->S_from_y = true; }
   if (s->pdrop_now) {
@@ -3605,7 +3672,7 @@
         hipGraph_t graph = nullptr;
         bool ok = hipStreamBeginCapture(s->stream, hipStreamCaptureModeRelaxed) == hipSuccess;
         if (ok) {
-          for (int i = 0; i < s->graph_iters; i++) enq_iter();
+          enq_iters(s->graph_iters);
           ok = hipStreamEndCapture(s->stream, &graph) == hipSuccess && graph != nullptr;
         }
         if (ok) ok = hipGraphInstantiate(&s->graph_exec[ar], graph, nullptr, nullptr, 0) == hipSuccess;
@@ -3639,7 +3706,7 @@
       s->st_graph_batches++;
     } else if (left > 0) {
       const int64_t nb_it = std::min<int64_t>(left, eager_batch);
-      for (int64_t i = 0; i < nb_it; i++) enq_iter();
+      enq_iters(nb_it);
       HIPCK(s, hipGetLastError());
       planned += nb_it;
       s->st_eager_batches++;
@@ -3712,6 +3779,13 @@
     s->ring_k = c->ring_k; s->ring_n = c->ring_n; s->ring_unc = c->ring_unc; s->ring_latest = c->latest; s->ring_j0 = c->ring_j0;
     memcpy(s->ring_alpha, c->ring_alpha, sizeof s->ring_alpha);
   }
+  if (c->err == SDPLR_ERR_FUSED_BARRIER) {
+    (void)hipMemsetAsync(s->fused_bar, 0, SDPLR_GBAR_WORDS * sizeof(double), s->stream);
+    s->fused_fit = 0;
+    c->err = 0; c->done = 0;
+    (void)push(s);
+    return bail(fail(s, SDPLR_ERR_HIP, "inner_loop: the fused step + direction kernel timed out at its grid barrier (grid not co-resident)"));
+  }
   if (c->done) why = c->exit_reason;
   if (loop_fused && c->iters > 0 && c->err == 0 && why != EXIT_RELDELTA) {
     s->dirt_from = c->latest - 1;
@@ -3738,6 +3812,7 @@
   s->G_age = s->pdrop_now ? s->G_age + c->iters : 0;
   if (s->pdrop_now) s->st_pdrop++;
   if (s->ring_now) s->st_ring_loops++;
+  if (s->fused_now) s->st_fused_loops++;
   s->G_consistent = true;
   *Lio = c->L; *gnio = c->gnorm; *pnio = c->pvnorm;
   if (last_alpha) *last_alpha = c->alpha;
```

Measured after the change: 6342, median of 6. Within noise of the previous version (+0.5%).
